# google/yggdrasil-decision-forests

Measured on NVIDIA H100. Metric: GBT boosting iters/sec, 10M rows x 200 num feats, higher is better.
Workload: dtype int64 fixed-point sums (q24 gradients), f64 split scores

## Files before the change

include/ygg_b200.h:

```cpp
#ifndef YGG_B200_H_
#define YGG_B200_H_

#include <stdint.h>

#ifdef __cplusplus
extern "C" {
#endif

#define YGG_ABI_VERSION 3

enum ygg_status {
  YGG_OK = 0,
  YGG_ERR_INVALID_ARGUMENT = 1,
  YGG_ERR_NO_DEVICE = 2,
  YGG_ERR_CUDA = 3,
  YGG_ERR_UNIMPLEMENTED = 4,
  YGG_ERR_CANCELLED = 5,
  YGG_ERR_IO = 6
};

enum ygg_loss {
  YGG_LOSS_BINOMIAL_LOG_LIKELIHOOD = 0,
  YGG_LOSS_SQUARED_ERROR = 1,
  YGG_LOSS_MULTINOMIAL_LOG_LIKELIHOOD = 2
// ... 40 lines not shown
  YGG_FEATURE_DISCRETIZED_NUMERICAL = 0,
  YGG_FEATURE_CATEGORICAL = 1,
  YGG_FEATURE_NUMERICAL = 2
};

typedef struct ygg_node {
  int32_t feature;
  int32_t threshold_bin;
  int32_t na_value;
  int32_t depth;
  int32_t neg_child;
  int32_t pos_child;
  float split_score;
  float leaf_value;
  int64_t num_examples;
  int64_t num_pos_examples;
  double stat[3];
  int32_t condition_type;
  float threshold_value;
  uint32_t cat_mask[8];
} ygg_node;

typedef struct ygg_dataset ygg_dataset;
typedef struct ygg_gbt ygg_gbt;

int ygg_abi_version(void);
const char* ygg_last_error(void);
int ygg_device_count(void);

int ygg_dataset_create(ygg_dataset** out, int64_t n_rows, int32_t n_features,
                       const uint8_t* bins, int64_t column_stride,
                       const int32_t* num_bins, const int32_t* na_bin, int32_t device);
int ygg_dataset_set_feature_types(ygg_dataset* ds, const int32_t* feature_types, int32_t n_features);
int ygg_dataset_set_bucket_values(ygg_dataset* ds, int32_t feature, const float* values, int32_t n, float na_replacement);
int ygg_dataset_set_wide_column(ygg_dataset* ds, int32_t feature, const uint16_t* codes, int64_t n, int32_t num_bins, int32_t na_bin,
                                const float* values, float na_replacement);
int ygg_dataset_set_wide_categorical_column(ygg_dataset* ds, int32_t feature, const uint16_t* codes, int64_t n, int32_t num_bins,
                                            int32_t na_bin);
int ygg_dataset_set_wide_discretized_column(ygg_dataset* ds, int32_t feature, const uint16_t* codes, int64_t n, int32_t num_bins,
                                            int32_t na_bin);
int ygg_dataset_get_wide_column(const ygg_dataset* ds, int32_t feature, uint16_t* codes, int32_t* num_bins, int32_t* na_bin);
int ygg_dataset_set_numerical_column(ygg_dataset* ds, int32_t feature, const float* values, int64_t n, float na_replacement);
int ygg_dataset_get_numerical_column(const ygg_dataset* ds, int32_t feature, float* values);
int ygg_dataset_destroy(ygg_dataset* ds);
int64_t ygg_dataset_num_rows(const ygg_dataset* ds);
int32_t ygg_dataset_num_features(const ygg_dataset* ds);

void ygg_gbt_config_init(ygg_gbt_config* cfg);
int ygg_gbt_create(ygg_gbt** out, ygg_dataset* ds, const ygg_gbt_config* cfg);
int ygg_gbt_destroy(ygg_gbt* h);

int ygg_gbt_set_labels_i32(ygg_gbt* h, const int32_t* labels, int64_t n);
int ygg_gbt_set_labels_f32(ygg_gbt* h, const float* labels, int64_t n);

int ygg_gbt_set_weights_f32(ygg_gbt* h, const float* weights, int64_t n);

int ygg_validation_split_mask(uint32_t random_seed, int64_t n_rows, float validation_ratio,
                              uint8_t* out_in_training );
int ygg_dataset_split_rows(const ygg_dataset* ds, const uint8_t* select, ygg_dataset** selected,
                           ygg_dataset** rest);
int ygg_gbt_set_validation_i32(ygg_gbt* h, const ygg_dataset* valid, const int32_t* labels, int64_t n);
int ygg_gbt_set_validation_f32(ygg_gbt* h, const ygg_dataset* valid, const float* labels, int64_t n);
int ygg_gbt_set_validation_weights_f32(ygg_gbt* h, const float* weights, int64_t n);
int ygg_gbt_validation_loss(ygg_gbt* h, int32_t iter, float* loss, float* secondary);
int32_t ygg_gbt_num_iterations(const ygg_gbt* h);
int ygg_gbt_final_validation(ygg_gbt* h, float* validation_loss, int32_t* early_stopping_triggered);

typedef int (*ygg_allgather_fn)(void* ctx, const void* send, void* recv, int64_t bytes,
                                void* stream);
int ygg_gbt_set_feature_shard(ygg_gbt* h, int32_t feature_begin, int32_t feature_end,
                              int32_t rank, int32_t world, ygg_allgather_fn exchange, void* ctx);

typedef int (*ygg_allreduce_fn)(void* ctx, void* buf, int64_t count, int32_t dtype, int32_t op, void* stream);
int ygg_gbt_set_row_shard(ygg_gbt* h, int32_t rank, int32_t world, int64_t n_rows_global,
                          float initial_prediction, ygg_allreduce_fn allreduce, void* ctx);

typedef int (*ygg_reducescatter_fn)(void* ctx, void* buf, int64_t count_per_rank, int32_t dtype, int32_t op,
                                    void* stream);
int ygg_gbt_set_row_shard_scatter(ygg_gbt* h, int32_t rank, int32_t world, int64_t n_rows_global,
                                  float initial_prediction, ygg_allreduce_fn allreduce,
                                  ygg_reducescatter_fn reducescatter, ygg_allgather_fn allgather, void* ctx);

int ygg_feature_shard(int32_t n_features, int32_t rank, int32_t world, int32_t* begin, int32_t* end);

typedef struct ygg_shard_best {
  float score;
  int32_t feature;
  int32_t threshold_bin;
  int32_t num_pos_examples;
  int32_t condition_type;
  int32_t na_value;
  uint32_t cat_mask[8];
} ygg_shard_best;
int ygg_merge_shard_best(const ygg_shard_best* records, int32_t world, int32_t nodes, ygg_shard_best* out);

int ygg_gbt_initial_prediction(ygg_gbt* h, float* out);

int ygg_gbt_train(ygg_gbt* h, int32_t num_iters, const volatile int32_t* stop_flag);
int ygg_gbt_step(ygg_gbt* h);
int ygg_gbt_sync(ygg_gbt* h);

int ygg_gbt_train_timed(ygg_gbt* h, int32_t num_iters, double* device_ms, int64_t* kernel_launches);

int32_t ygg_gbt_num_trees(const ygg_gbt* h);
int64_t ygg_gbt_best_split_window_bytes(const ygg_gbt* h);
int ygg_gbt_set_best_split_window(ygg_gbt* h, void* const* peer_windows, int32_t world);

int ygg_gbt_tie_stats(ygg_gbt* h, int64_t* renamed, int64_t* unresolved);
int ygg_gbt_set_tie_rng_position(ygg_gbt* h, uint64_t words);

int ygg_num_candidate_attributes(int32_t num_features, int32_t loss, int32_t num_candidate_attributes,
                                 float num_candidate_attributes_ratio, int32_t* k);
uint64_t ygg_candidate_key(uint32_t random_seed, int32_t tree, int32_t node, int32_t feature);
int ygg_gbt_set_candidate_sampling(ygg_gbt* h, int32_t num_candidate_attributes, float num_candidate_attributes_ratio);

int ygg_gbt_set_dart(ygg_gbt* h, float dropout_rate);
int ygg_gbt_get_dart_weights(ygg_gbt* h, float* out, int32_t capacity, int32_t* n);
int ygg_gbt_get_dart_dropped(ygg_gbt* h, int32_t iter, int32_t* out, int32_t capacity, int32_t* n);

int ygg_gbt_get_tree(ygg_gbt* h, int32_t iter, ygg_node* out, int32_t capacity, int32_t* n_nodes);
int ygg_gbt_get_category_set(ygg_gbt* h, int32_t iter, int32_t node, uint32_t* words, int32_t capacity, int32_t* n_words);
int ygg_gbt_train_loss(ygg_gbt* h, int32_t iter, float* loss, float* secondary);
int ygg_gbt_get_predictions(ygg_gbt* h, float* out, int64_t n);
int ygg_gbt_predict(ygg_gbt* h, const ygg_dataset* ds, float* out, int64_t n);

int ygg_gbt_set_predictions(ygg_gbt* h, const float* pred, int64_t n);

int ygg_tree_train_on_gradients(ygg_gbt* h, const float* gradients, const float* hessians,
                                ygg_node* out, int32_t capacity, int32_t* n_nodes);

enum ygg_hist_mode {
  YGG_HIST_ROOT_SUM = 0,
  YGG_HIST_PACKED = 1,
  YGG_HIST_SHARED = 2,
  YGG_HIST_HIST2 = 3,
  YGG_HIST_SEGMENTED = 4,
};
typedef struct ygg_hist_plan {
  int32_t mode;
  int32_t group;
  union {
    int32_t hist2_tiles;
    int32_t root_lanes;
  };
  int32_t chunk_blocks;
  int32_t slot_window;
  int32_t grid;
} ygg_hist_plan;
int ygg_debug_hist_plan(const ygg_gbt* h, int32_t level, ygg_hist_plan* out);
int ygg_debug_level_histogram(ygg_gbt* h, int32_t level, const ygg_hist_plan* plan, const float* gradients,
                              const float* second, const int32_t* slot_of_row, int32_t n_slots, uint64_t* out_sum,
                              uint32_t* out_cnt, uint64_t* out_second, float* out_scales);

int ygg_debug_wide_histogram(ygg_gbt* h, int32_t n_slots, uint64_t* out_sum, uint32_t* out_cnt, uint64_t* out_second);

int ygg_debug_capture_candidates(ygg_gbt* h, int32_t enabled);
typedef struct ygg_level_node {
  int32_t node;
  int32_t candidate;
  int32_t derived;
  int32_t reserved;
  int64_t num_examples;
} ygg_level_node;
typedef struct ygg_candidate {
  int32_t found;
  float score;
  int32_t threshold_bin;
  int32_t lo, hi;
  int32_t num_pos_examples;
  float threshold_value;
  uint32_t cat_mask[8];
} ygg_candidate;
int ygg_debug_level_candidates(ygg_gbt* h, int32_t level, int32_t capacity, ygg_level_node* nodes, ygg_candidate* cands,
                               uint32_t* sets, int32_t set_words, int32_t* n_nodes, float* scales);
int ygg_debug_level_tried(ygg_gbt* h, int32_t level, int32_t capacity, uint8_t* tried, int32_t* first_node, int32_t* n_nodes);

int ygg_partition_rows(ygg_dataset* ds, const uint32_t* rows_in, int64_t n, int32_t feature,
                       int32_t threshold_bin, uint32_t* rows_out, int64_t* n_pos);

int ygg_gbt_set_profiling(ygg_gbt* h, int32_t enabled);
int ygg_gbt_get_profile(ygg_gbt* h, const char* name, double* ms, int64_t* launches);

int ygg_gbt_save_ydf(ygg_gbt* h, const char* directory, const char* label_name,
                     const uint8_t* data_spec_pb, int64_t data_spec_len, int32_t label_col_idx,
                     const int32_t* feature_col_idx);

#ifdef __cplusplus
}
#endif
#endif
```

yggdrasil-decision-forests_b200/_capi.py:

```python
import ctypes as C
import os

import numpy as np

from . import _build

_LIB = None


class YggError(RuntimeError):
    def __init__(self, code, msg):
        super().__init__(f"[ygg status {code}] {msg}")
        self.code = code


class GbtConfig(C.Structure):
    _fields_ = [
        ("abi_version", C.c_int32), ("loss", C.c_int32), ("num_trees", C.c_int32),
        ("shrinkage", C.c_float), ("max_depth", C.c_int32), ("min_examples", C.c_int32),
        ("in_split_min_examples_check", C.c_int32), ("use_hessian_gain", C.c_int32),
        ("l1_regularization", C.c_float), ("l2_regularization", C.c_float),
        ("l2_regularization_categorical", C.c_float), ("clamp_leaf_logit", C.c_float),
        ("hessian_split_score_subtract_parent", C.c_int32), ("random_seed", C.c_uint32),
        ("subsample", C.c_float), ("validation_ratio", C.c_float),
        ("sibling_subtraction", C.c_int32), ("early_stopping", C.c_int32),
        ("early_stopping_num_trees_look_ahead", C.c_int32), ("early_stopping_initial_iteration", C.c_int32),
        ("num_classes", C.c_int32), ("candidate_shuffle", C.c_int32), ("rng_words_consumed", C.c_uint32),
        ("split_jobs_draw_seeds", C.c_int32), ("growing_strategy", C.c_int32), ("max_num_nodes", C.c_int32),
        ("goss_alpha", C.c_float), ("goss_beta", C.c_float),
    ]


NODE_DTYPE = np.dtype([
    ("feature", "<i4"), ("threshold_bin", "<i4"), ("na_value", "<i4"), ("depth", "<i4"),
    ("neg_child", "<i4"), ("pos_child", "<i4"), ("split_score", "<f4"), ("leaf_value", "<f4"),
    ("num_examples", "<i8"), ("num_pos_examples", "<i8"), ("stat", "<f8", (3,)),
    ("condition_type", "<i4"), ("threshold_value", "<f4"), ("cat_mask", "<u4", (8,)),
])
assert NODE_DTYPE.itemsize == 112

FEATURE_DISCRETIZED_NUMERICAL = 0
FEATURE_CATEGORICAL = 1
FEATURE_NUMERICAL = 2

LEVEL_NODE_DTYPE = np.dtype([("node", "<i4"), ("candidate", "<i4"), ("derived", "<i4"), ("reserved", "<i4"),
                             ("num_examples", "<i8")])
assert LEVEL_NODE_DTYPE.itemsize == 24
CANDIDATE_DTYPE = np.dtype([("found", "<i4"), ("score", "<f4"), ("threshold_bin", "<i4"), ("lo", "<i4"), ("hi", "<i4"),
                            ("num_pos_examples", "<i4"), ("threshold_value", "<f4"), ("cat_mask", "<u4", (8,))])
assert CANDIDATE_DTYPE.itemsize == 60

HIST_ROOT_SUM, HIST_PACKED, HIST_SHARED, HIST2, HIST_SEGMENTED = 0, 1, 2, 3, 4


class HistPlan(C.Structure):
    _fields_ = [("mode", C.c_int32), ("group", C.c_int32), ("hist2_tiles", C.c_int32), ("chunk_blocks", C.c_int32),
                ("slot_window", C.c_int32), ("grid", C.c_int32)]

    root_lanes = property(lambda self: self.hist2_tiles, lambda self, v: setattr(self, "hist2_tiles", v))

    def __repr__(self):
        return "HistPlan(%s)" % ", ".join("%s=%d" % (k, getattr(self, k)) for k, _ in self._fields_)

ALLGATHER_FN = C.CFUNCTYPE(C.c_int, C.c_void_p, C.c_void_p, C.c_void_p, C.c_int64, C.c_void_p)
ALLREDUCE_FN = C.CFUNCTYPE(C.c_int, C.c_void_p, C.c_void_p, C.c_int64, C.c_int32, C.c_int32, C.c_void_p)
REDUCESCATTER_FN = C.CFUNCTYPE(C.c_int, C.c_void_p, C.c_void_p, C.c_int64, C.c_int32, C.c_int32, C.c_void_p)

EXPORTS = [
    "ygg_abi_version", "ygg_last_error", "ygg_device_count", "ygg_dataset_create",
    "ygg_dataset_set_feature_types", "ygg_dataset_destroy", "ygg_dataset_num_rows", "ygg_dataset_num_features",
    "ygg_gbt_config_init", "ygg_gbt_create", "ygg_gbt_destroy", "ygg_gbt_set_labels_i32",
    "ygg_gbt_set_labels_f32", "ygg_gbt_set_weights_f32", "ygg_gbt_set_validation_weights_f32", "ygg_gbt_set_feature_shard", "ygg_gbt_set_row_shard", "ygg_gbt_set_row_shard_scatter", "ygg_feature_shard",
    "ygg_merge_shard_best", "ygg_gbt_initial_prediction",
    "ygg_gbt_train", "ygg_gbt_train_timed", "ygg_gbt_step", "ygg_gbt_sync", "ygg_gbt_num_trees", "ygg_gbt_get_tree",
    "ygg_gbt_train_loss", "ygg_gbt_get_predictions", "ygg_gbt_set_predictions", "ygg_gbt_predict",
    "ygg_tree_train_on_gradients", "ygg_debug_hist_plan", "ygg_debug_level_histogram", "ygg_partition_rows",
    "ygg_gbt_set_profiling", "ygg_gbt_get_profile", "ygg_gbt_save_ydf",
    "ygg_discretize_boundaries", "ygg_discretize_encode", "ygg_model_write_ydf",
    "ygg_validation_split_mask", "ygg_dataset_split_rows", "ygg_gbt_set_validation_i32",
    "ygg_gbt_set_validation_f32", "ygg_gbt_validation_loss", "ygg_gbt_num_iterations", "ygg_gbt_final_validation",
    "ygg_gen_discretized_boundaries", "ygg_dataset_builder_create", "ygg_dataset_builder_add_numerical",
    "ygg_dataset_builder_add_numerical_async", "ygg_dataset_builder_get_numerical",
    "ygg_dataset_builder_add_bins", "ygg_dataset_builder_finish", "ygg_dataset_builder_destroy",
    "ygg_dataset_get_bins", "ygg_dataset_set_bucket_values", "ygg_gbt_tie_stats", "ygg_gbt_set_tie_rng_position",
    "ygg_gbt_best_split_window_bytes", "ygg_gbt_set_best_split_window", "ygg_comm_window_create",
    "ygg_comm_unique_id", "ygg_comm_create", "ygg_comm_destroy", "ygg_comm_allreduce", "ygg_comm_allgather", "ygg_comm_reducescatter",
    "ygg_dataset_set_wide_column", "ygg_dataset_get_wide_column", "ygg_debug_wide_histogram",
    "ygg_dataset_set_wide_categorical_column", "ygg_gbt_get_category_set",
    "ygg_dataset_set_numerical_column", "ygg_dataset_get_numerical_column",
    "ygg_debug_capture_candidates", "ygg_debug_level_candidates",
    "ygg_num_candidate_attributes", "ygg_candidate_key", "ygg_gbt_set_candidate_sampling", "ygg_debug_level_tried",
    "ygg_gbt_set_dart", "ygg_gbt_get_dart_weights", "ygg_gbt_get_dart_dropped",
    "ygg_dataset_set_wide_discretized_column", "ygg_dataset_builder_add_numerical16_async", "ygg_discretize_boundaries16",
]


def lib():
    global _LIB
    if _LIB is None:
        path = _build.build()
        L = C.CDLL(path)
        L.ygg_last_error.restype = C.c_char_p
        L.ygg_dataset_num_rows.restype = C.c_int64
        L.ygg_gbt_config_init.restype = None
        L.ygg_candidate_key.restype = C.c_uint64
        L.ygg_candidate_key.argtypes = [C.c_uint32, C.c_int32, C.c_int32, C.c_int32]
        for name in EXPORTS:
            getattr(L, name)
        _LIB = L
    return _LIB


def check(status):
    if status != 0:
        raise YggError(status, lib().ygg_last_error().decode("utf-8", "replace"))


def ptr(a, t):
    return a.ctypes.data_as(C.POINTER(t)) if a is not None else None


def num_candidate_attributes(num_features, loss, num_candidate_attributes=-1, ratio=None):
    k = C.c_int32()
    check(lib().ygg_num_candidate_attributes(C.c_int32(int(num_features)), C.c_int32(int(loss)),
                                             C.c_int32(int(num_candidate_attributes)),
                                             C.c_float(-1.0 if ratio is None else float(ratio)), C.byref(k)))
    return k.value


def candidate_key(seed, tree, node, feature):
    return int(lib().ygg_candidate_key(int(seed) & 0xFFFFFFFF, int(tree), int(node), int(feature)))


def default_config(**kw):
    cfg = GbtConfig()
    lib().ygg_gbt_config_init(C.byref(cfg))
    for k, v in kw.items():
        if not hasattr(cfg, k):
            raise AttributeError(k)
        setattr(cfg, k, v)
    return cfg


class Dataset:

    def __init__(self, bins, num_bins, na_bin, device=0, feature_types=None):
        b = np.asarray(bins)
        if not (b.dtype == np.uint8 and b.ndim == 2 and b.strides[1] == 1 and b.strides[0] >= b.shape[1]):
            b = np.ascontiguousarray(bins, dtype=np.uint8)
        assert b.ndim == 2, "bins must be [n_features, n_rows] (column-major storage)"
        self.n_features, self.n_rows = b.shape
        self.num_bins = np.ascontiguousarray(num_bins, dtype=np.int32)
        self.na_bin = np.ascontiguousarray(na_bin, dtype=np.int32)
        assert len(self.num_bins) == self.n_features and len(self.na_bin) == self.n_features
        self.handle = C.c_void_p()
        self.h2d_bytes = self.n_features * self.n_rows
        col_stride = b.strides[0] if self.n_features > 1 else max(int(b.strides[0]), self.n_rows)
        check(lib().ygg_dataset_create(C.byref(self.handle), C.c_int64(self.n_rows),
                                       C.c_int32(self.n_features), C.cast(b.ctypes.data, C.POINTER(C.c_uint8)),
                                       C.c_int64(col_stride), ptr(self.num_bins, C.c_int32),
                                       ptr(self.na_bin, C.c_int32), C.c_int32(device)))
        self.feature_types = np.zeros(self.n_features, np.int32)
        if feature_types is not None:
            self.set_feature_types(feature_types)

    def set_bucket_values(self, feature, values, na_replacement):
        v = np.ascontiguousarray(values, dtype=np.float32)
        check(lib().ygg_dataset_set_bucket_values(self.handle, C.c_int32(int(feature)), ptr(v, C.c_float), C.c_int32(len(v)),
                                                  C.c_float(float(np.float32(na_replacement)))))

    def set_wide_column(self, feature, codes, num_bins, na_bin, values, na_replacement):
        c = np.ascontiguousarray(codes, dtype=np.uint16)
        v = np.ascontiguousarray(values, dtype=np.float32)
        if len(v) != int(num_bins):
            raise ValueError(f"{len(v)} bucket values for {num_bins} buckets")
        check(lib().ygg_dataset_set_wide_column(self.handle, C.c_int32(int(feature)), ptr(c, C.c_uint16), C.c_int64(len(c)),
                                                C.c_int32(int(num_bins)), C.c_int32(int(na_bin)), ptr(v, C.c_float),
                                                C.c_float(float(np.float32(na_replacement)))))
        self.num_bins = self.num_bins.copy()
        self.na_bin = self.na_bin.copy()
        self.num_bins[feature], self.na_bin[feature] = 1, 0
        self.wide = dict(getattr(self, "wide", {}))
        self.wide[int(feature)] = (int(num_bins), int(na_bin))

    def set_wide_categorical_column(self, feature, codes, num_bins, na_bin):
        c = np.ascontiguousarray(codes, dtype=np.uint16)
        check(lib().ygg_dataset_set_wide_categorical_column(self.handle, C.c_int32(int(feature)), ptr(c, C.c_uint16),
                                                            C.c_int64(len(c)), C.c_int32(int(num_bins)), C.c_int32(int(na_bin))))
        self.num_bins = self.num_bins.copy()
        self.na_bin = self.na_bin.copy()
        self.num_bins[feature], self.na_bin[feature] = 1, 0
        self.wide = dict(getattr(self, "wide", {}))
        self.wide[int(feature)] = (int(num_bins), int(na_bin))

    def set_wide_discretized_column(self, feature, codes, num_bins, na_bin):
        c = np.ascontiguousarray(codes, dtype=np.uint16)
        check(lib().ygg_dataset_set_wide_discretized_column(self.handle, C.c_int32(int(feature)), ptr(c, C.c_uint16),
                                                            C.c_int64(len(c)), C.c_int32(int(num_bins)), C.c_int32(int(na_bin))))
        self.num_bins = self.num_bins.copy()
        self.na_bin = self.na_bin.copy()
        self.num_bins[feature], self.na_bin[feature] = 1, 0
        self.wide = dict(getattr(self, "wide", {}))
        self.wide[int(feature)] = (int(num_bins), int(na_bin))

    def get_wide_column(self, feature):
        out = np.empty(self.n_rows, np.uint16)
        nb, na = C.c_int32(), C.c_int32()
        check(lib().ygg_dataset_get_wide_column(self.handle, C.c_int32(int(feature)), ptr(out, C.c_uint16), C.byref(nb), C.byref(na)))
        return out, nb.value, na.value

    def set_numerical_column(self, feature, values, na_replacement):
        v = np.ascontiguousarray(values, dtype=np.float32)
        check(lib().ygg_dataset_set_numerical_column(self.handle, C.c_int32(int(feature)), ptr(v, C.c_float), C.c_int64(len(v)),
                                                     C.c_float(float(np.float32(na_replacement)))))
        self.num_bins = self.num_bins.copy()
        self.na_bin = self.na_bin.copy()
        self.num_bins[feature], self.na_bin[feature] = 1, 0
        self.feature_types = self.feature_types.copy()
        self.feature_types[feature] = FEATURE_NUMERICAL

    def get_numerical_column(self, feature):
        out = np.empty(self.n_rows, np.float32)
        check(lib().ygg_dataset_get_numerical_column(self.handle, C.c_int32(int(feature)), ptr(out, C.c_float)))
        return out

    def set_feature_types(self, feature_types):
        ft = np.ascontiguousarray(feature_types, dtype=np.int32)
        check(lib().ygg_dataset_set_feature_types(self.handle, ptr(ft, C.c_int32), C.c_int32(len(ft))))
        self.feature_types = ft

    def close(self):
        if self.handle:
            lib().ygg_dataset_destroy(self.handle)
            self.handle = C.c_void_p()

    def split_rows(self, select):
        m = np.ascontiguousarray(select, dtype=np.uint8)
        assert m.shape == (self.n_rows,)
        a, b = C.c_void_p(), C.c_void_p()
        check(lib().ygg_dataset_split_rows(self.handle, ptr(m, C.c_uint8), C.byref(a), C.byref(b)))
        out = []
        for hnd, n in ((a, int(m.astype(bool).sum())), (b, int(len(m) - m.astype(bool).sum()))):
            d = Dataset.__new__(Dataset)
            d.handle, d.n_features, d.n_rows = hnd, self.n_features, n
            d.num_bins, d.na_bin, d.feature_types, d.h2d_bytes = self.num_bins, self.na_bin, self.feature_types, 0
            d.wide = dict(getattr(self, "wide", {}))
# ... 278 lines not shown
                        return int(fn(*a) or 0)
                    except Exception:
                        import traceback
                        traceback.print_exc()
                        return 1
                return _cb
            self._cbs = (ALLREDUCE_FN(wrap(allreduce, 5)), REDUCESCATTER_FN(wrap(reducescatter, 5)),
                         ALLGATHER_FN(wrap(allgather, 4)))
            fns, ctx = self._cbs, None
        check(lib().ygg_gbt_set_row_shard_scatter(self.handle, C.c_int32(rank), C.c_int32(world),
                                                  C.c_int64(n_rows_global), C.c_float(initial_prediction),
                                                  fns[0], fns[1], fns[2], ctx))

    def set_row_shard(self, rank, world, n_rows_global, initial_prediction, allreduce=None):
        if isinstance(allreduce, Comm):
            self._comm = allreduce
            fn = C.cast(lib().ygg_comm_allreduce, ALLREDUCE_FN)
            check(lib().ygg_gbt_set_row_shard(self.handle, C.c_int32(rank), C.c_int32(world),
                                              C.c_int64(n_rows_global), C.c_float(initial_prediction), fn,
                                              allreduce.handle))
            return
        if allreduce is not None:
            def _cb(ctx, buf, count, dtype, op, stream):
                try:
                    return int(allreduce(buf, count, dtype, op, stream) or 0)
                except Exception:
                    import traceback
                    traceback.print_exc()
                    return 1
            self._cb = ALLREDUCE_FN(_cb)
            fn = self._cb
        else:
            fn = C.cast(None, ALLREDUCE_FN)
        check(lib().ygg_gbt_set_row_shard(self.handle, C.c_int32(rank), C.c_int32(world),
                                          C.c_int64(n_rows_global), C.c_float(initial_prediction), fn, None))

    def initial_prediction(self):
        v = C.c_float()
        check(lib().ygg_gbt_initial_prediction(self.handle, C.byref(v)))
        return v.value

    def train(self, num_iters, stop_flag=None):
        check(lib().ygg_gbt_train(self.handle, C.c_int32(num_iters), stop_flag))

    def train_timed(self, num_iters):
        ms, n = C.c_double(), C.c_int64()
        check(lib().ygg_gbt_train_timed(self.handle, C.c_int32(num_iters), C.byref(ms), C.byref(n)))
        return ms.value, n.value

    def step(self):
        check(lib().ygg_gbt_step(self.handle))

    def sync(self):
        check(lib().ygg_gbt_sync(self.handle))

    def num_trees(self):
        return int(lib().ygg_gbt_num_trees(self.handle))

    def use_peer_windows(self, comm):
        L = lib()
        L.ygg_gbt_best_split_window_bytes.restype = C.c_int64
        nbytes = int(L.ygg_gbt_best_split_window_bytes(self.handle))
        peers = (C.c_void_p * comm.world)()
        check(L.ygg_comm_window_create(comm.handle, C.c_int64(nbytes), peers))
        check(L.ygg_gbt_set_best_split_window(self.handle, peers, C.c_int32(comm.world)))

    def set_tie_rng_position(self, words):
        check(lib().ygg_gbt_set_tie_rng_position(self.handle, C.c_uint64(int(words))))

    def tie_stats(self):
        a, b = C.c_int64(), C.c_int64()
        check(lib().ygg_gbt_tie_stats(self.handle, C.byref(a), C.byref(b)))
        return a.value, b.value

    def get_tree(self, it):
        cap = (1 << (self.cfg.max_depth + (1 if self.cfg.growing_strategy == 1 else 0)))
        out = np.zeros(cap, dtype=NODE_DTYPE)
        n = C.c_int32()
        check(lib().ygg_gbt_get_tree(self.handle, C.c_int32(it), out.ctypes.data_as(C.c_void_p),
                                     C.c_int32(cap), C.byref(n)))
        return out[:n.value].copy()

    def get_category_sets(self, it, tree=None):
        wide = getattr(self.dataset, "wide", {})
        if not wide:
            return {}
        t = self.get_tree(it) if tree is None else tree
        out = {}
        for i in np.flatnonzero((t["condition_type"] == FEATURE_CATEGORICAL) & (t["feature"] >= 0)):
            f = int(t["feature"][i])
            if f not in wide:
                continue
            words = np.zeros((wide[f][0] + 31) // 32, np.uint32)
            n = C.c_int32()
            check(lib().ygg_gbt_get_category_set(self.handle, C.c_int32(it), C.c_int32(int(i)), ptr(words, C.c_uint32),
                                                 C.c_int32(len(words)), C.byref(n)))
            out[int(i)] = words
        return out

    def train_loss(self, it):
        a, b = C.c_float(), C.c_float()
        check(lib().ygg_gbt_train_loss(self.handle, C.c_int32(it), C.byref(a), C.byref(b)))
        return a.value, b.value

    def get_predictions(self):
        k = self.cfg.num_classes if self.cfg.loss == 2 else 1
        out = np.empty(self.dataset.n_rows * k, dtype=np.float32)
        check(lib().ygg_gbt_get_predictions(self.handle, ptr(out, C.c_float), C.c_int64(len(out))))
        return out if k == 1 else np.ascontiguousarray(out.reshape(k, self.dataset.n_rows).T)

    def predict(self, dataset):
        n = int(lib().ygg_dataset_num_rows(dataset.handle))
        K = int(self.cfg.num_classes) if self.cfg.loss == 2 else 1
        out = np.empty(n * K, dtype=np.float32)
        check(lib().ygg_gbt_predict(self.handle, dataset.handle, ptr(out, C.c_float), C.c_int64(n * K)))
        return out if K == 1 else np.ascontiguousarray(out.reshape(K, n).T)

    def set_predictions(self, pred):
        p = np.ascontiguousarray(pred, dtype=np.float32)
        check(lib().ygg_gbt_set_predictions(self.handle, ptr(p, C.c_float), C.c_int64(len(p))))

    def train_tree_on_gradients(self, g, h=None):
        g = np.ascontiguousarray(g, dtype=np.float32)
        h = None if h is None else np.ascontiguousarray(h, dtype=np.float32)
        cap = (1 << (self.cfg.max_depth + (1 if self.cfg.growing_strategy == 1 else 0)))
        out = np.zeros(cap, dtype=NODE_DTYPE)
        n = C.c_int32()
        check(lib().ygg_tree_train_on_gradients(self.handle, ptr(g, C.c_float), ptr(h, C.c_float),
                                                out.ctypes.data_as(C.c_void_p), C.c_int32(cap),
                                                C.byref(n)))
        return out[:n.value].copy()

    def hist_plan(self, level):
        p = HistPlan()
        check(lib().ygg_debug_hist_plan(self.handle, C.c_int32(level), C.byref(p)))
        return p

    def level_histogram(self, level, g, slot_of_row, n_slots, second=None, plan=None):
        g = np.ascontiguousarray(g, dtype=np.float32)
        slots = np.ascontiguousarray(slot_of_row, dtype=np.int32)
        v = None if second is None else np.ascontiguousarray(second, dtype=np.float32)
        lo, hi = self.hist_features()
        shape = (int(n_slots), hi - lo, 256)
        s = np.zeros(shape, np.uint64)
        c = np.zeros(shape, np.uint32)
        s2 = None if v is None else np.zeros(shape, np.uint64)
        scales = np.zeros(2, np.float32)
        check(lib().ygg_debug_level_histogram(self.handle, C.c_int32(level), None if plan is None else C.byref(plan),
                                              ptr(g, C.c_float), ptr(v, C.c_float), ptr(slots, C.c_int32),
                                              C.c_int32(n_slots), ptr(s, C.c_uint64), ptr(c, C.c_uint32),
                                              ptr(s2, C.c_uint64), ptr(scales, C.c_float)))
        return s, c, s2, (float(scales[0]), float(scales[1]))

    def wide_histogram(self, n_slots):
        total = sum(nb for nb, _ in getattr(self.dataset, "wide", {}).values())
        s = np.zeros((int(n_slots), total), np.uint64)
        c = np.zeros((int(n_slots), total), np.uint32)
        s2 = np.zeros((int(n_slots), total), np.uint64) if self.has_second_plane() else None
        check(lib().ygg_debug_wide_histogram(self.handle, C.c_int32(int(n_slots)), ptr(s, C.c_uint64), ptr(c, C.c_uint32),
                                             ptr(s2, C.c_uint64)))
        return s, c, s2

    def has_second_plane(self):
        weighted = getattr(self, "_weighted", False) or self.cfg.goss_alpha > 0 or self.cfg.goss_beta > 0
        logit = self.cfg.loss in (0, 2)
        return bool((self.cfg.use_hessian_gain and (logit or weighted)) or weighted)

    def debug_histogram(self, g, node_of_row, node, feature):
        lo, hi = self.hist_features()
        if not lo <= feature < hi:
            raise ValueError(f"feature {feature} outside the histogrammed features [{lo}, {hi})")
        slots = np.where(np.asarray(node_of_row) == node, 0, -1).astype(np.int32)
        root = self.hist_plan(0)
        p = HistPlan(HIST_SHARED, 1, 0, root.chunk_blocks, 0, root.grid)
        second = np.zeros(len(slots), np.float32) if self.has_second_plane() else None
        s, c, _, (P, _) = self.level_histogram(0, g, slots, 1, second=second, plan=p)
        nb = int(self.dataset.num_bins[feature])
        cnt = c[0, feature - lo, :nb].astype(np.int64)
        raw = s[0, feature - lo, :nb].astype(np.int64) - cnt * 2 ** 23
        return raw.astype(np.float64) * (P / 2.0 ** 23), cnt

    def set_candidate_sampling(self, num_candidate_attributes=-1, ratio=None):
        check(lib().ygg_gbt_set_candidate_sampling(self.handle, C.c_int32(int(num_candidate_attributes)),
                                                   C.c_float(-1.0 if ratio is None else float(ratio))))

    def set_dart(self, dropout_rate):
        check(lib().ygg_gbt_set_dart(self.handle, C.c_float(float(dropout_rate))))

    def dart_weights(self):
        n = C.c_int32()
        cap = int(self.cfg.num_trees)
        out = np.zeros(max(cap, 1), np.float32)
        check(lib().ygg_gbt_get_dart_weights(self.handle, ptr(out, C.c_float), C.c_int32(cap), C.byref(n)))
        return out[:n.value].copy()

    def dart_dropped(self, it):
        n = C.c_int32()
        out = np.zeros(max(int(it), 1), np.int32)
        check(lib().ygg_gbt_get_dart_dropped(self.handle, C.c_int32(int(it)), ptr(out, C.c_int32), C.c_int32(len(out)),
                                             C.byref(n)))
        return out[:n.value].copy()

    def level_tried(self, level):
        cap = 1 << max(0, self.cfg.max_depth - 1)
        lo, hi = self.hist_features()
        out = np.zeros((cap, hi - lo), np.uint8)
        first, n = C.c_int32(), C.c_int32()
        check(lib().ygg_debug_level_tried(self.handle, C.c_int32(int(level)), C.c_int32(cap), ptr(out, C.c_uint8),
                                          C.byref(first), C.byref(n)))
        return out[:n.value].copy(), first.value

    def capture_candidates(self, on=True):
        check(lib().ygg_debug_capture_candidates(self.handle, C.c_int32(int(bool(on)))))

    def level_candidates(self, level):
        cap = 1 << max(0, self.cfg.max_depth - 1)
        lo, hi = self.hist_features()
        nodes = np.zeros(cap, LEVEL_NODE_DTYPE)
        cands = np.zeros((cap, hi - lo), CANDIDATE_DTYPE)
        wide = getattr(self.dataset, "wide", {})
        words = max([(nb + 31) // 32 for f, (nb, _) in wide.items()
                     if self.dataset.feature_types[f] == FEATURE_CATEGORICAL] or [0])
        sets = np.zeros((cap, len(wide), words), np.uint32) if words else None
        n, scales = C.c_int32(), np.zeros(3, np.float32)
        check(lib().ygg_debug_level_candidates(self.handle, C.c_int32(int(level)), C.c_int32(cap),
                                               nodes.ctypes.data_as(C.c_void_p), cands.ctypes.data_as(C.c_void_p),
                                               ptr(sets, C.c_uint32), C.c_int32(words), C.byref(n), ptr(scales, C.c_float)))
        k = n.value
        out = {name: nodes[name][:k].copy() for name in ("node", "candidate", "derived", "num_examples")}
        out.update({name: cands[name][:k].copy() for name in CANDIDATE_DTYPE.names})
        if sets is not None:
            out["sets"] = sets[:k].copy()
        out["P"], out["h_pow2"], out["w_pow2"] = (float(x) for x in scales)
        return out

    def hist_features(self):
        return getattr(self, "_hist_features", (0, self.dataset.n_features))

    def set_profiling(self, enabled=True):
        check(lib().ygg_gbt_set_profiling(self.handle, C.c_int32(int(enabled))))

    def get_profile(self, name):
        ms, n = C.c_double(), C.c_int64()
        check(lib().ygg_gbt_get_profile(self.handle, name.encode(), C.byref(ms), C.byref(n)))
        return ms.value, n.value


SHARD_BEST_DTYPE = np.dtype([("score", "<f4"), ("feature", "<i4"), ("threshold_bin", "<i4"),
                             ("num_pos_examples", "<i4"), ("condition_type", "<i4"), ("na_value", "<i4"),
                             ("cat_mask", "<u4", (8,))])
assert SHARD_BEST_DTYPE.itemsize == 56


def feature_shard(n_features, rank, world):
    b, e = C.c_int32(), C.c_int32()
    check(lib().ygg_feature_shard(C.c_int32(n_features), C.c_int32(rank), C.c_int32(world),
                                  C.byref(b), C.byref(e)))
    return b.value, e.value


def merge_shard_best(records):
    r = np.ascontiguousarray(records, dtype=SHARD_BEST_DTYPE)
    world, nodes = r.shape
    out = np.zeros(nodes, dtype=SHARD_BEST_DTYPE)
    check(lib().ygg_merge_shard_best(r.ctypes.data_as(C.c_void_p), C.c_int32(world), C.c_int32(nodes),
                                     out.ctypes.data_as(C.c_void_p)))
    return out


def device_count():
    return int(lib().ygg_device_count())


def discretize_boundaries(values, maximum_num_bins=255, min_obs_in_bins=3):
    v = np.ascontiguousarray(values, dtype=np.float32)
    out = np.zeros(max(2, maximum_num_bins + 4), dtype=np.float32)
    n = C.c_int32()
    mean = C.c_double()
    check(lib().ygg_discretize_boundaries(ptr(v, C.c_float), C.c_int64(len(v)),
                                          C.c_int32(maximum_num_bins), C.c_int32(min_obs_in_bins),
                                          ptr(out, C.c_float), C.c_int32(len(out)), C.byref(n),
                                          C.byref(mean)))
    return out[:n.value].copy(), mean.value


def discretize_boundaries16(values, maximum_num_bins, min_obs_in_bins=3):
    v = np.ascontiguousarray(values, dtype=np.float32)
    out = np.zeros(maximum_num_bins + 4, dtype=np.float32)
    n = C.c_int32()
    mean = C.c_double()
    check(lib().ygg_discretize_boundaries16(ptr(v, C.c_float), C.c_int64(len(v)),
                                            C.c_int32(maximum_num_bins), C.c_int32(min_obs_in_bins),
                                            ptr(out, C.c_float), C.c_int32(len(out)), C.byref(n),
                                            C.byref(mean)))
    return out[:n.value].copy(), mean.value


def discretize_encode(values, boundaries, na_bin):
    v = np.ascontiguousarray(values, dtype=np.float32)
    b = np.ascontiguousarray(boundaries, dtype=np.float32)
    out = np.empty(len(v), dtype=np.uint8)
    check(lib().ygg_discretize_encode(ptr(v, C.c_float), C.c_int64(len(v)), ptr(b, C.c_float),
                                      C.c_int32(len(b)), C.c_int32(na_bin), ptr(out, C.c_uint8)))
    return out
```

yggdrasil-decision-forests_b200/csrc/ygg_engine.cu:

```cuda
#include <algorithm>
#include <mutex>
#include <random>
#include <cmath>
#include <cstdarg>
#include <cstdio>
#include <cstdlib>
#include <cstring>
#include <limits>
#include <map>
#include <queue>
#include <string>
#include <thread>
#include <vector>

#include <cuda_runtime.h>
#include <cub/device/device_radix_sort.cuh>
#include <cub/device/device_scan.cuh>
#include <nvtx3/nvToolsExt.h>

#include "../../include/ygg_b200.h"
#include "ygg_internal.h"
#include "../../include/ygg_b200_model.h"
#include "ygg_kernels.cuh"
#include "ygg_wide.cuh"
// ... 108 lines not shown
  float* d_pred = nullptr;
  float* d_g = nullptr;
  float* d_h = nullptr;
  uint32_t* d_q24 = nullptr;
  uint32_t* d_hq24 = nullptr;
  uint2* d_act = nullptr;
  uint32_t* d_act_h = nullptr;
  int32_t* d_act_count = nullptr;
  int32_t* d_act_sub = nullptr;
  uint32_t* d_root_cnt = nullptr;
  bool root_cnt_valid = false;
  int n_blocks = 0;
  uint16_t* d_node_of_row = nullptr;
  DeviceState* d_st = nullptr;
  LevelDesc* d_levels = nullptr;
  Family* d_fam[2] = {nullptr, nullptr};
  int32_t* d_slot_node[2] = {nullptr, nullptr};
  NodeRec* d_nodes_all = nullptr;
  NodeRec* d_nodes_scratch = nullptr;
  int tree_capacity = 0;
  unsigned long long* d_hist_sum[2] = {nullptr, nullptr};
  uint32_t* d_hist_cnt[2] = {nullptr, nullptr};
  unsigned long long* d_hist_hsum[2] = {nullptr, nullptr};
  Candidate* d_cand = nullptr;
  uint32_t* d_cand_mask = nullptr;
  int64_t wide_total = 0;
  int wide_slots = 0;
  bool counted = false;
  unsigned long long* d_wsum = nullptr;
  uint32_t* d_wcnt = nullptr;
  unsigned long long* d_whsum = nullptr;
  unsigned long long* d_wnode_sum[2] = {nullptr, nullptr};
  uint32_t* d_wnode_cnt[2] = {nullptr, nullptr};
  unsigned long long* d_wnode_hsum[2] = {nullptr, nullptr};
  float* d_wide_thr = nullptr;
  int32_t* d_wide_feature = nullptr;
  int32_t* d_wide_bins = nullptr;
  int32_t* d_wide_disc = nullptr;
  int set_words = 0;
  int64_t sort_total = 0;
  int64_t* d_sort_off = nullptr;
  int32_t* d_wide_cat = nullptr;
  int32_t* d_wide_na_bin = nullptr;
  uint32_t* d_wide_set = nullptr;
  double* d_sort_key = nullptr;
  int32_t* d_sort_idx = nullptr;
  uint32_t* d_sets = nullptr;
  float* d_master_val = nullptr;
  uint32_t* d_master_row = nullptr;
  float* d_list_val[2] = {nullptr, nullptr};
  uint32_t* d_list_row[2] = {nullptr, nullptr};
  unsigned long long* d_ps = nullptr;
  unsigned long long* d_ph = nullptr;
  int64_t* d_seg_off = nullptr;
  int64_t* d_seg_total = nullptr;
  unsigned long long* d_sbest = nullptr;
  unsigned long long* d_sbest_idx = nullptr;
  int32_t* d_num_feature = nullptr;
  void* d_presort_temp = nullptr;
  size_t presort_temp_bytes = 0;
  bool scratch_tree = false;
  ShardBest* d_shard_best = nullptr;
  TieRec* d_ties = nullptr;
  int sample_k_valid = 0;
  uint8_t* d_tried = nullptr;
  bool dart = false;
  float dart_rate = 0.f;
  uint16_t* d_dart_hist = nullptr;
  uint16_t* d_dart_vhist = nullptr;
  float* d_dart_leaf = nullptr;
  DartDrop* d_dart_list[2] = {nullptr, nullptr};
  std::vector<std::vector<int32_t>> dart_dropped;
  std::vector<float> dart_w_new, dart_sf_m1, dart_w;
  std::vector<DartDrop> dart_host_list;
  struct Capture {
    bool on = false;
    int levels = 0;
    const NodeRec* tree = nullptr;
    int f_scan = 0;
    size_t nodes = 0, set_elems = 0;
    Candidate* cand = nullptr;
    uint32_t* mask = nullptr;
    float* thr = nullptr;
    uint32_t* set = nullptr;
    uint8_t* tried = nullptr;
    NodeRec* node_tab = nullptr;
    Family* fam = nullptr;
    LevelDesc* lv = nullptr;
    DeviceState* st = nullptr;
  } cap;
  uint8_t* d_selected = nullptr;
  std::vector<uint8_t> host_selected;
  int64_t n_selected = 0;
  std::mt19937 tie_rng;
  bool tie_rng_ready = false;
  int ties_resolved_upto = 0;
  int64_t ties_renamed = 0, ties_unresolved = 0;
  LossRec* d_loss = nullptr;
  LossPartials* d_loss_partials = nullptr;
  unsigned long long* d_level_buf = nullptr;
  size_t level_buf_bytes = 0;
  size_t slot_elems_cap = 0;
  int stats_cap = 0;
  int shard_mode = kShardNone;
  int hist_f_begin = 0, hist_f_end = 0;
  int64_t n_global = 0;
  ygg_allreduce_fn allreduce = nullptr;
  ygg_reducescatter_fn reducescatter = nullptr;
  bool scatter = false;
  int loss_reduced_upto = 0;
  int max_nodes = 0, max_level_nodes = 0, num_levels = 0;
  int trees_done = 0;
  bool pending = false;
  int K = 1;
  int iters_done = 0;
  bool pending_loss = false;
  float* cur_g = nullptr;
  float* cur_h = nullptr;
  float* cur_g2w = nullptr;
  const ygg_dataset* vds = nullptr;
  float* d_vpred = nullptr;
  uint8_t* d_vlabel_u8 = nullptr;
  float* d_vlabel_f32 = nullptr;
  LossRec* d_vloss = nullptr;
  float* d_weight = nullptr;
  float* d_g2w = nullptr;
  unsigned long long* d_wsums = nullptr;
  std::vector<float> host_weights;
  double sum_weights = 0;
  float w_pow2 = 1.f;
  float* d_goss_keys[2] = {nullptr, nullptr};
  uint32_t* d_goss_rows[2] = {nullptr, nullptr};
  float* d_goss_u = nullptr;
  void* d_goss_temp = nullptr;
  size_t goss_temp_bytes = 0;
  std::vector<float> host_goss_u;
  int64_t goss_cutoff = 0;
  float* d_vweight = nullptr;
  double v_sum_weights = 0;
  float v_correct_scale = 0.f;
  bool finalized = false;
  int final_trees = -1;
  int log_entries = -1;
  float final_validation_loss = 0.f;
  bool early_stopping_triggered = false;
  int f_begin = 0, f_end = 0, rank = 0, world = 1;
  ygg_allgather_fn exchange = nullptr;
  void* exchange_ctx = nullptr;
  void** d_peer_windows = nullptr;
  uint32_t exchange_epoch = 0;
  HistLaunch hist_plan[32]{};
  int part_smem_children = 0;
  uint2* d_hseg = nullptr;
  long long* d_hseg_blk = nullptr;
  long long* d_hseg_off = nullptr;
  int32_t* d_hseg_piece = nullptr;
  int32_t* d_hseg_meta = nullptr;
  void* d_hseg_temp = nullptr;
  size_t hseg_temp_bytes = 0;
  bool profiling = false;
  std::map<std::string, ProfileSlot> profile;
  std::vector<std::pair<std::string, std::pair<cudaEvent_t, cudaEvent_t>>> pending_events;
  int64_t launches_total = 0;
};

namespace {

bool use_hess(const ygg_gbt* h) { return h->cfg.use_hessian_gain != 0; }
bool is_logit(const ygg_gbt* h) {
  return h->cfg.loss == YGG_LOSS_BINOMIAL_LOG_LIKELIHOOD || h->cfg.loss == YGG_LOSS_MULTINOMIAL_LOG_LIKELIHOOD;
}
bool is_multinomial(const ygg_gbt* h) { return h->cfg.loss == YGG_LOSS_MULTINOMIAL_LOG_LIKELIHOOD; }
bool weighted(const ygg_gbt* h) { return h->d_weight != nullptr; }
bool has_h(const ygg_gbt* h) { return is_logit(h) || weighted(h); }
float h_pow2_of(const ygg_gbt* h) { return (is_logit(h) ? 0.25f : 1.f) * (weighted(h) ? h->w_pow2 : 1.f); }
float correct_scale_of(float w_pow2) { return static_cast<float>(1u << kSBits) / w_pow2; }
bool hist_hess(const ygg_gbt* h) { return (use_hess(h) && has_h(h)) || weighted(h); }
bool goss(const ygg_gbt* h) { return h->cfg.goss_alpha > 0.f || h->cfg.goss_beta > 0.f; }
bool sampling(const ygg_gbt* h) { return h->cfg.subsample < 1.f - std::numeric_limits<float>::epsilon() || goss(h); }
bool user_weighted(const ygg_gbt* h) { return h->d_weight != nullptr && !goss(h); }

inline bool nvtx_enabled() {
  static const bool on = [] { const char* v = std::getenv("YGG_NVTX"); return v != nullptr && std::atoi(v) != 0; }();
  return on;
}
struct ProfScope {
  ygg_gbt* h;
  const char* name;
  cudaEvent_t a = nullptr, b = nullptr;
  ProfScope(ygg_gbt* h_, const char* n) : h(h_), name(n) {
    if (nvtx_enabled()) nvtxRangePushA(n);
    if (h->profiling) {
      cudaEventCreate(&a);
      cudaEventCreate(&b);
      cudaEventRecord(a, h->stream);
    }
  }
  ~ProfScope() {
    if (h->profiling) {
      cudaEventRecord(b, h->stream);
      h->pending_events.push_back({name, {a, b}});
    }
    if (nvtx_enabled()) nvtxRangePop();
  }
};

void collect_profile(ygg_gbt* h) {
  for (auto& e : h->pending_events) {
    float ms = 0;
    cudaEventSynchronize(e.second.second);
    cudaEventElapsedTime(&ms, e.second.first, e.second.second);
    auto& s = h->profile[e.first];
    s.ms += ms;
    s.launches++;
    cudaEventDestroy(e.second.first);
    cudaEventDestroy(e.second.second);
  }
  h->pending_events.clear();
}

int check_launch(const char* what) {
  cudaError_t e = cudaGetLastError();
  if (e != cudaSuccess) return set_error(YGG_ERR_CUDA, "launch of %s failed: %s", what, cudaGetErrorString(e));
  return YGG_OK;
}

int level_slot_bound(const ygg_gbt* h, int level) {
  if (level == 0) return 1;
  return h->cfg.sibling_subtraction ? (1 << (level - 1)) : (1 << level);
}

struct LevelBuf {
  unsigned long long* sum;
  unsigned long long* hsum;
  uint32_t* cnt;
  unsigned long long* stats;
  int W;
  int f_chunk;
  size_t chunk_u64;
  size_t planes_u64;
  size_t total_u64;
};
LevelBuf level_buf(const ygg_gbt* h, int slots, int n_stats_nodes, unsigned long long* base = nullptr) {
  LevelBuf lb;
  const int f_hist = h->hist_f_end - h->hist_f_begin;
  lb.W = h->scatter ? h->world : 1;
  lb.f_chunk = (f_hist + lb.W - 1) / lb.W;
  const size_t B = static_cast<size_t>(slots) * lb.f_chunk * kMaxBins;
  if (base == nullptr) base = h->d_level_buf;
  lb.sum = base;
  unsigned long long* p = lb.sum + B;
  lb.hsum = nullptr;
  if (hist_hess(h)) { lb.hsum = p; p += B; }
  lb.cnt = reinterpret_cast<uint32_t*>(p);
  p += (B + 1) / 2;
  lb.stats = p;
  lb.planes_u64 = static_cast<size_t>(p - base);
  p += static_cast<size_t>(n_stats_nodes) * 3;
  lb.chunk_u64 = static_cast<size_t>(p - base);
  lb.total_u64 = lb.chunk_u64 * lb.W;
  return lb;
}

__global__ void k_zero_planes(unsigned long long* base, size_t chunk_u64, size_t planes_u64) {
  unsigned long long* c = base + static_cast<size_t>(blockIdx.y) * chunk_u64;
  for (size_t i = static_cast<size_t>(blockIdx.x) * blockDim.x + threadIdx.x; i < planes_u64;
       i += static_cast<size_t>(gridDim.x) * blockDim.x)
    c[i] = 0ull;
}
__global__ void k_replicate_stats(unsigned long long* stats0, size_t chunk_u64, int n_words, int W) {
  const int i = blockIdx.x * blockDim.x + threadIdx.x;
  if (i >= n_words) return;
  const unsigned long long v = stats0[i];
  for (int c = 1; c < W; c++) stats0[static_cast<size_t>(c) * chunk_u64 + i] = v;
}

int zero_planes(ygg_gbt* h, const LevelBuf& lb) {
  if (lb.W == 1) {
    YGG_CUDA(cudaMemsetAsync(lb.sum, 0, lb.planes_u64 * sizeof(unsigned long long), h->stream));
    return YGG_OK;
  }
  dim3 grid(static_cast<unsigned>(std::min<size_t>((lb.planes_u64 + 255) / 256, 1024)), static_cast<unsigned>(lb.W));
  k_zero_planes<<<grid, 256, 0, h->stream>>>(lb.sum, lb.chunk_u64, lb.planes_u64);
  h->launches_total++;
  return check_launch("k_zero_planes");
}
int replicate_stats(ygg_gbt* h, const LevelBuf& lb, int n_nodes) {
  if (lb.W == 1) return YGG_OK;
  k_replicate_stats<<<(3 * n_nodes + 127) / 128, 128, 0, h->stream>>>(lb.stats, lb.chunk_u64, 3 * n_nodes, lb.W);
  h->launches_total++;
  return check_launch("k_replicate_stats");
}

template <typename F>
int for_hist_kernel(bool hess, int mode, F f, bool multi = false) {
  if (multi) {
    if (hess) return f(k_hist<true, kHistShared, true>);
    if (mode == kHistPacked) return f(k_hist<false, kHistPacked, true>);
    return f(k_hist<false, kHistShared, true>);
  }
  if (hess) return f(k_hist<true, kHistShared>);
  if (mode == kHistRootSum) return f(k_hist<false, kHistRootSum>);
  if (mode == kHistPacked) return f(k_hist<false, kHistPacked>);
  return f(k_hist<false, kHistShared>);
}

int hist_smem_budget(int device, size_t* budget) {
  int optin = 0;
  YGG_CUDA(cudaDeviceGetAttribute(&optin, cudaDevAttrMaxSharedMemoryPerBlockOptin, device));
  cudaFuncAttributes fa{};
  YGG_CUDA(cudaFuncGetAttributes(&fa, k_hist<false, kHistPacked>));
  *budget = static_cast<size_t>(optin) - fa.sharedSizeBytes;
  return YGG_OK;
}
constexpr size_t kHist2SmemBudget = 216 * 1024;

int sub_blocks_of(const ygg_gbt* h) { return h->ds->n_pad / kBlockRows >= 512 ? 8 : 1; }
int chunk_max_count(ygg_gbt* h, int chunk_blocks, uint32_t** d_sub, uint32_t* out_max) {
  const int kSubBlocks = sub_blocks_of(h);
  const ygg_dataset* ds = h->ds;
  const int f_count = h->hist_f_end - h->hist_f_begin;
  const int n_blocks = static_cast<int>(ds->n_pad / kBlockRows);
  const int n_subs = (n_blocks + kSubBlocks - 1) / kSubBlocks;
  if (*d_sub == nullptr) {
    YGG_RETURN_IF_ERROR(dev_alloc(d_sub, static_cast<size_t>(n_subs) * f_count * kMaxBins + 1));
    k_sub_counts<<<dim3(n_subs, f_count), 256>>>(ds->d_bins, ds->n, ds->n_pad, h->hist_f_begin, kSubBlocks, *d_sub);
    YGG_RETURN_IF_ERROR(check_launch("k_sub_counts"));
  }
  uint32_t* d_max = *d_sub + static_cast<size_t>(n_subs) * f_count * kMaxBins;
  YGG_CUDA(cudaMemset(d_max, 0, sizeof(uint32_t)));
  const int subs_per_chunk = chunk_blocks / kSubBlocks;
  const int n_chunks = (n_subs + subs_per_chunk - 1) / subs_per_chunk;
  k_chunk_max<<<dim3(n_chunks, f_count), 256>>>(*d_sub, n_subs, subs_per_chunk, d_max);
  YGG_CUDA(cudaMemcpy(out_max, d_max, sizeof(uint32_t), cudaMemcpyDeviceToHost));
  return YGG_OK;
}

int raise_hist_smem_caps_once(int device) {
  static std::mutex mu;
  static std::vector<char> done;
  std::lock_guard<std::mutex> lock(mu);
  if (static_cast<int>(done.size()) <= device) done.resize(device + 1, 0);
  if (done[device]) return YGG_OK;
  size_t budget = 0;
  YGG_RETURN_IF_ERROR(hist_smem_budget(device, &budget));
  auto set_cap = [](size_t bytes) {
    return [bytes](auto kern) -> int {
      YGG_CUDA(cudaFuncSetAttribute(kern, cudaFuncAttributeMaxDynamicSharedMemorySize, static_cast<int>(bytes)));
      return YGG_OK;
    };
  };
  for (const bool hess : {false, true})
    for (const int mode : {kHistRootSum, kHistPacked, kHistShared})
      for (const bool multi : {false, true}) YGG_RETURN_IF_ERROR(for_hist_kernel(hess, mode, set_cap(budget), multi));
  const auto cap2 = set_cap(kHist2SmemBudget);
  YGG_RETURN_IF_ERROR(cap2(k_hist2<32, true>)); YGG_RETURN_IF_ERROR(cap2(k_hist2<32, false>));
  YGG_RETURN_IF_ERROR(cap2(k_hist2<16, true>)); YGG_RETURN_IF_ERROR(cap2(k_hist2<16, false>));
  YGG_RETURN_IF_ERROR(cap2(k_hist2<8, true>)); YGG_RETURN_IF_ERROR(cap2(k_hist2<8, false>));
  YGG_RETURN_IF_ERROR(set_cap(seg_smem_bytes(64))(k_hist_seg<32, 2>));
  YGG_RETURN_IF_ERROR(set_cap(seg_smem_bytes(32))(k_hist_seg<32, 1>));
  YGG_RETURN_IF_ERROR(set_cap(seg_smem_bytes(16))(k_hist_seg<16, 1>));
  YGG_RETURN_IF_ERROR(set_cap(seg_smem_bytes(8))(k_hist_seg<8, 1>));
  YGG_CUDA(cudaFuncSetAttribute(k_hist_seg<32, 2>, cudaFuncAttributePreferredSharedMemoryCarveout, cudaSharedmemCarveoutMaxShared));
  YGG_CUDA(cudaFuncSetAttribute(k_hist_seg<32, 1>, cudaFuncAttributePreferredSharedMemoryCarveout, cudaSharedmemCarveoutMaxShared));
  YGG_CUDA(cudaFuncSetAttribute(k_hist_seg<16, 1>, cudaFuncAttributePreferredSharedMemoryCarveout, cudaSharedmemCarveoutMaxShared));
  YGG_CUDA(cudaFuncSetAttribute(k_hist_seg<8, 1>, cudaFuncAttributePreferredSharedMemoryCarveout, cudaSharedmemCarveoutMaxShared));
  YGG_RETURN_IF_ERROR(set_cap(kRootSmemBytes)(k_hist_root_rows));
  done[device] = 1;
  return YGG_OK;
}

int configure_launches(ygg_gbt* h) {
  (void)cudaGetLastError();
  const bool hh = hist_hess(h);
  size_t budget = 0;
// ... 267 lines not shown
                                             h->d_master_row + static_cast<int64_t>(p) * n, static_cast<int>(n), 0, 32, h->stream));
  YGG_CUDA(cudaStreamSynchronize(h->stream));
  return YGG_OK;
}

PresortParams presort_params(ygg_gbt* h, NodeRec* nodes, int l, const ScanParams& sc) {
  const ygg_dataset* ds = h->ds;
  PresortParams p{};
  p.s = sc; p.level = l; p.P = ds->n_num(); p.n = ds->n; p.num_feature = h->d_num_feature;
  const bool master = l == 0 && !sampling(h);
  p.val = master ? h->d_master_val : h->d_list_val[l & 1];
  p.row = master ? h->d_master_row : h->d_list_row[l & 1];
  p.s.nodes = nodes; p.s.levels = h->d_levels;
  p.node_of_row = h->d_node_of_row; p.seg_off = h->d_seg_off; p.seg_total = h->d_seg_total;
  p.q24 = h->d_q24; p.hq24 = hist_hess(h) ? h->d_hq24 : nullptr; p.ps = h->d_ps; p.ph = h->d_ph;
  p.best = h->d_sbest; p.best_idx = h->d_sbest_idx; p.thr_value = h->d_wide_thr;
  return p;
}

int presort_scan(ygg_gbt* h, const PresortParams& p) {
  const int64_t total = static_cast<int64_t>(p.P) * p.n;
  const int grid = elementwise_grid(h);
  if (p.level == 0) {
    k_presort_segments<<<1, 1024, 0, h->stream>>>(h->d_levels, p.s.nodes, 0, h->d_seg_off, h->d_seg_total);
    h->launches_total++;
    YGG_RETURN_IF_ERROR(check_launch("k_presort_segments"));
    if (sampling(h)) {
      uint32_t* flags = reinterpret_cast<uint32_t*>(h->d_ps);
      k_presort_sample_flags<<<grid, 256, 0, h->stream>>>(h->d_master_row, total, h->d_selected, flags);
      YGG_CUDA(cub::DeviceScan::ExclusiveSum(h->d_presort_temp, h->presort_temp_bytes, flags, flags, total, h->stream));
      k_presort_sample_scatter<<<grid, 256, 0, h->stream>>>(h->d_master_val, h->d_master_row, p.n, total, h->d_selected, flags,
                                                            h->d_list_val[0], h->d_list_row[0]);
      h->launches_total += 3;
      YGG_RETURN_IF_ERROR(check_launch("k_presort_sample_scatter"));
    }
  }
  k_presort_gather<<<grid, 256, 0, h->stream>>>(p);
  YGG_CUDA(cub::DeviceScan::InclusiveSum(h->d_presort_temp, h->presort_temp_bytes, h->d_ps, h->d_ps, total, h->stream));
  if (p.hq24 != nullptr)
    YGG_CUDA(cub::DeviceScan::InclusiveSum(h->d_presort_temp, h->presort_temp_bytes, h->d_ph, h->d_ph, total, h->stream));
  const size_t slots = (static_cast<size_t>(1) << p.level) * p.P;
  YGG_CUDA(cudaMemsetAsync(h->d_sbest, 0, slots * sizeof(unsigned long long), h->stream));
  YGG_CUDA(cudaMemsetAsync(h->d_sbest_idx, 0xFF, slots * sizeof(unsigned long long), h->stream));
  if (hist_hess(h) || use_hess(h)) {
    k_presort_scan<true, true><<<grid, 256, 0, h->stream>>>(p);
    k_presort_scan<true, false><<<grid, 256, 0, h->stream>>>(p);
  } else {
    k_presort_scan<false, true><<<grid, 256, 0, h->stream>>>(p);
    k_presort_scan<false, false><<<grid, 256, 0, h->stream>>>(p);
  }
  k_presort_candidates<<<static_cast<unsigned>((slots + 255) / 256), 256, 0, h->stream>>>(p);
  h->launches_total += 5 + (p.hq24 != nullptr ? 1 : 0);
  return check_launch("k_presort_candidates");
}

int presort_partition(ygg_gbt* h, NodeRec* nodes, int l) {
  ScanParams sc{};
  PresortParams p = presort_params(h, nodes, l, sc);
  const int64_t total = static_cast<int64_t>(p.P) * p.n;
  const int grid = elementwise_grid(h);
  k_presort_segments<<<1, 1024, 0, h->stream>>>(h->d_levels, nodes, l + 1, h->d_seg_off, h->d_seg_total);
  uint32_t* flags = reinterpret_cast<uint32_t*>(h->d_ps);
  k_presort_flags<<<grid, 256, 0, h->stream>>>(p, flags);
  YGG_CUDA(cub::DeviceScan::ExclusiveSum(h->d_presort_temp, h->presort_temp_bytes, flags, flags, total, h->stream));
  k_presort_scatter<<<grid, 256, 0, h->stream>>>(p, flags, h->d_list_val[(l + 1) & 1], h->d_list_row[(l + 1) & 1]);
  h->launches_total += 4;
  return check_launch("k_presort_scatter");
}

int allocate_level_buffers(ygg_gbt* h) {
  const int f_scan = h->f_end - h->f_begin;
  const int f_hist = h->hist_f_end - h->hist_f_begin;
  for (int i = 0; i < 2; i++) {
    dev_free(h->d_hist_sum[i]); dev_free(h->d_hist_cnt[i]); dev_free(h->d_hist_hsum[i]);
    h->d_hist_sum[i] = nullptr; h->d_hist_cnt[i] = nullptr; h->d_hist_hsum[i] = nullptr;
  }
  dev_free(h->d_cand); h->d_cand = nullptr;
  dev_free(h->d_cand_mask); h->d_cand_mask = nullptr;
  cudaFree(h->d_level_buf); h->d_level_buf = nullptr;
  const size_t split_level_nodes = static_cast<size_t>(1) << std::max(0, h->num_levels - 1);
  const size_t node_elems = split_level_nodes * f_scan * kMaxBins;
  for (int i = 0; i < 2; i++) {
    YGG_RETURN_IF_ERROR(dev_alloc(&h->d_hist_sum[i], node_elems));
    YGG_RETURN_IF_ERROR(dev_alloc(&h->d_hist_cnt[i], node_elems));
    if (hist_hess(h)) YGG_RETURN_IF_ERROR(dev_alloc(&h->d_hist_hsum[i], node_elems));
  }
  YGG_RETURN_IF_ERROR(dev_alloc(&h->d_cand, split_level_nodes * f_scan));
  YGG_RETURN_IF_ERROR(dev_alloc(&h->d_cand_mask, split_level_nodes * f_scan * 8));
  if (h->d_shard_best == nullptr)
    YGG_RETURN_IF_ERROR(dev_alloc_plain(&h->d_shard_best, static_cast<size_t>(std::max(1, h->world)) * h->max_level_nodes));
  size_t max_u64 = 16;
  for (int l = 0; l <= h->num_levels; l++) {
    const int slots = l < h->num_levels ? level_slot_bound(h, l) : 0;
    const int stats_nodes = l == 0 ? 1 : (2 << (l - 1));
    max_u64 = std::max(max_u64, level_buf(h, slots, stats_nodes).total_u64);
  }
  (void)f_hist;
  h->level_buf_bytes = max_u64 * sizeof(unsigned long long);
  YGG_RETURN_IF_ERROR(dev_alloc_plain(&h->d_level_buf, max_u64));
  return allocate_wide_buffers(h);
}

int launch_hist(ygg_gbt* h, const HistParams& hp, int mode, int grid, size_t smem, bool multi = false) {
  return for_hist_kernel(hist_hess(h), mode, [&](auto kern) -> int {
    kern<<<grid, kHistThreads, smem, h->stream>>>(hp);
    h->launches_total++;
    return check_launch("k_hist");
  }, multi);
}

int ensure_bins4(ygg_dataset* ds) {
  if (ds->d_bins4 != nullptr) return YGG_OK;
  const int groups = (ds->F + 3) / 4;
  YGG_RETURN_IF_ERROR(dev_alloc(&ds->d_bins4, static_cast<size_t>(groups) * ds->n_pad));
  dim3 grid(static_cast<unsigned>(std::min<int64_t>((ds->n_pad / 4 + 255) / 256, 4096)), static_cast<unsigned>(groups));
  k_interleave4<<<grid, 256>>>(ds->d_bins, ds->n_pad, ds->F, ds->d_bins4);
  YGG_RETURN_IF_ERROR(check_launch("k_interleave4"));
  YGG_CUDA(cudaDeviceSynchronize());
  return YGG_OK;
}

int launch_hist2(ygg_gbt* h, const Hist2Params& hp, int FL, bool root, int grid) {
  const size_t smem = hist2_smem_bytes(FL, hp.S, hp.T, root);
  auto go = [&](auto kern) -> int {
    kern<<<grid, kHist2Threads, smem, h->stream>>>(hp);
    h->launches_total++;
    return check_launch("k_hist2");
  };
  if (FL == 32) return root ? go(k_hist2<32, true>) : go(k_hist2<32, false>);
  if (FL == 16) return root ? go(k_hist2<16, true>) : go(k_hist2<16, false>);
  return root ? go(k_hist2<8, true>) : go(k_hist2<8, false>);
}

int ensure_bins_rows(ygg_dataset* ds) {
  static std::mutex mu;
  std::lock_guard<std::mutex> lock(mu);
  if (ds->d_bins_rows != nullptr) return YGG_OK;
  const int row_bytes = seg_row_bytes(ds->F);
  uint8_t* rows = nullptr;
  YGG_RETURN_IF_ERROR(dev_alloc(&rows, static_cast<size_t>(row_bytes) * ds->n_pad));
  dim3 grid(static_cast<unsigned>((ds->n_pad + 255) / 256), static_cast<unsigned>(row_bytes / 32));
  k_bins_to_rows<<<grid, 256>>>(ds->d_bins, ds->n_pad, ds->F, row_bytes, rows);
  int st = check_launch("k_bins_to_rows");
  if (st == YGG_OK && cudaDeviceSynchronize() != cudaSuccess) st = set_error(YGG_ERR_CUDA, "k_bins_to_rows failed");
  if (st != YGG_OK) {
    dev_free(rows);
    return st;
  }
  ds->d_bins_rows = rows;
  return YGG_OK;
}

void free_seg_buffers(ygg_gbt* h) {
  dev_free(h->d_hseg); dev_free(h->d_hseg_blk); dev_free(h->d_hseg_off); dev_free(h->d_hseg_piece); dev_free(h->d_hseg_meta);
  dev_free(h->d_hseg_temp);
  h->d_hseg = nullptr; h->d_hseg_blk = nullptr; h->d_hseg_off = nullptr; h->d_hseg_piece = nullptr; h->d_hseg_meta = nullptr;
  h->d_hseg_temp = nullptr;
  h->hseg_temp_bytes = 0;
}
int ensure_seg_buffers(ygg_gbt* h) {
  if (h->d_hseg_temp != nullptr) return YGG_OK;
  const size_t ranges = static_cast<size_t>(kSegMaxSlots) * h->n_blocks;
  auto alloc_all = [&]() -> int {
    YGG_RETURN_IF_ERROR(dev_alloc(&h->d_hseg, static_cast<size_t>(h->ds->n_pad)));
    YGG_RETURN_IF_ERROR(dev_alloc(&h->d_hseg_blk, ranges));
    YGG_RETURN_IF_ERROR(dev_alloc(&h->d_hseg_off, ranges + 1));
    YGG_RETURN_IF_ERROR(dev_alloc(&h->d_hseg_piece, ranges + 1));
    YGG_RETURN_IF_ERROR(dev_alloc(&h->d_hseg_meta, 4));
    size_t temp_bytes = 0;
    YGG_CUDA(cub::DeviceScan::InclusiveSum(nullptr, temp_bytes, h->d_hseg_blk, h->d_hseg_blk, static_cast<int>(ranges)));
    char* temp = nullptr;
    YGG_RETURN_IF_ERROR(dev_alloc(&temp, temp_bytes));
    h->hseg_temp_bytes = temp_bytes;
    h->d_hseg_temp = temp;
    return YGG_OK;
  };
  const int st = alloc_all();
  if (st != YGG_OK) free_seg_buffers(h);
  return st;
}

int launch_hist_seg(ygg_gbt* h, int l, const LevelBuf& lb, const LevelDesc* levels, const HistLaunch& pl) {
  ygg_dataset* ds = h->ds;
  YGG_RETURN_IF_ERROR(ensure_bins_rows(ds));
  YGG_RETURN_IF_ERROR(ensure_seg_buffers(h));
  const int f_count = h->hist_f_end - h->hist_f_begin;
  const int n_chunks = (h->n_blocks + pl.chunk - 1) / pl.chunk;
  const int fpl = seg_lane_features(pl.SL, f_count);
  const int n_fg = seg_feature_groups(pl.SL, fpl, h->hist_f_begin, f_count);
  const int target_pieces = std::max(1, (kSegItemsPerCta * pl.grid + n_fg - 1) / n_fg);
  k_seg_count<<<std::min(h->n_blocks, ds->num_sms * 8), 256, 0, h->stream>>>(h->d_act, h->d_act_count, h->n_blocks, pl.S,
                                                                               levels, l, h->d_hseg_blk);
  YGG_RETURN_IF_ERROR(check_launch("k_seg_count"));
  YGG_CUDA(cub::DeviceScan::InclusiveSum(h->d_hseg_temp, h->hseg_temp_bytes, h->d_hseg_blk, h->d_hseg_blk, pl.S * h->n_blocks,
                                         h->stream));
  k_seg_ranges<<<1, kSegScanThreads, 0, h->stream>>>(h->d_hseg_blk, pl.S, h->n_blocks, pl.chunk, n_chunks, target_pieces,
                                                     h->d_hseg_off, h->d_hseg_piece, h->d_hseg_meta);
  YGG_RETURN_IF_ERROR(check_launch("k_seg_ranges"));
  k_seg_scatter<<<std::min(h->n_blocks, ds->num_sms * 8), 256, 0, h->stream>>>(h->d_act, h->d_act_count, h->n_blocks, pl.S, levels, l,
                                                               h->d_hseg_blk, h->d_hseg);
  YGG_RETURN_IF_ERROR(check_launch("k_seg_scatter"));
  SegParams sp{};
  sp.rows = ds->d_bins_rows; sp.row_bytes = static_cast<uint32_t>(seg_row_bytes(ds->F));
  sp.seg = h->d_hseg; sp.seg_off = h->d_hseg_off; sp.piece_start = h->d_hseg_piece; sp.meta = h->d_hseg_meta;
  sp.n_ranges = pl.S * n_chunks; sp.n_chunks = n_chunks;
  sp.f_begin = h->hist_f_begin; sp.f_count = f_count;
  sp.hist_sum = lb.sum; sp.hist_cnt = lb.cnt;
  sp.f_chunk = lb.f_chunk; sp.chunk_stride = static_cast<long long>(lb.chunk_u64);
  const size_t smem = seg_smem_bytes(pl.SL * fpl);
  if (fpl == 2) k_hist_seg<32, 2><<<pl.grid, kSegThreads, smem, h->stream>>>(sp);
  else if (pl.SL == 32) k_hist_seg<32, 1><<<pl.grid, kSegThreads, smem, h->stream>>>(sp);
  else if (pl.SL == 16) k_hist_seg<16, 1><<<pl.grid, kSegThreads, smem, h->stream>>>(sp);
  else k_hist_seg<8, 1><<<pl.grid, kSegThreads, smem, h->stream>>>(sp);
  h->launches_total += 5;
  return check_launch("k_hist_seg");
}

int launch_hist_root_rows(ygg_gbt* h, const LevelBuf& lb, const HistLaunch& pl) {
  ygg_dataset* ds = h->ds;
  YGG_RETURN_IF_ERROR(ensure_bins_rows(ds));
  RootRowsParams rp{};
  rp.rows = ds->d_bins_rows; rp.row_bytes = static_cast<uint32_t>(seg_row_bytes(ds->F));
  rp.q24 = h->d_q24; rp.act_count = h->d_act_count; rp.n_blocks = h->n_blocks; rp.chunk_blocks = pl.chunk;
  rp.f_begin = h->hist_f_begin; rp.f_count = h->hist_f_end - h->hist_f_begin;
  rp.hist_sum = lb.sum; rp.f_chunk = lb.f_chunk; rp.chunk_stride = static_cast<long long>(lb.chunk_u64);
  k_hist_root_rows<<<pl.grid, kRootThreads, kRootSmemBytes, h->stream>>>(rp);
  h->launches_total++;
  return check_launch("k_hist_root_rows");
}

int ensure_root_counts(ygg_gbt* h) {
  if (h->root_cnt_valid) return YGG_OK;
  const int f_count = h->hist_f_end - h->hist_f_begin;
  if (h->d_root_cnt) dev_free(h->d_root_cnt);
  h->d_root_cnt = nullptr;
  const LevelBuf lb = level_buf(h, 1, 1);
  const size_t padded = static_cast<size_t>(lb.W) * lb.f_chunk * kMaxBins;
  YGG_RETURN_IF_ERROR(dev_alloc(&h->d_root_cnt, padded));
  YGG_CUDA(cudaMemsetAsync(h->d_root_cnt, 0, padded * sizeof(uint32_t), h->stream));
  dim3 grid(std::max(1, h->ds->num_sms * 8 / std::max(1, f_count)), f_count);
  k_root_counts<<<grid, 256, 0, h->stream>>>(h->ds->d_bins, h->ds->n, h->ds->n_pad, f_count, h->hist_f_begin, h->d_root_cnt);
  h->launches_total++;
  YGG_RETURN_IF_ERROR(check_launch("k_root_counts"));
  h->root_cnt_valid = true;
  return YGG_OK;
}

int accumulate_level(ygg_gbt* h, int l, const LevelBuf& lb, const LevelDesc* levels, const HistLaunch& pl) {
  const ygg_dataset* ds = h->ds;
  const int hist_f_count = h->hist_f_end - h->hist_f_begin;
  YGG_RETURN_IF_ERROR(zero_planes(h, lb));
  if (pl.mode == kHistRootSum) {
    const size_t row = static_cast<size_t>(lb.f_chunk) * kMaxBins * sizeof(uint32_t);
    YGG_CUDA(cudaMemcpy2DAsync(lb.cnt, lb.chunk_u64 * sizeof(unsigned long long), h->d_root_cnt, row, row, lb.W,
                               cudaMemcpyDeviceToDevice, h->stream));
  }
  if (pl.SL > 0) return launch_hist_seg(h, l, lb, levels, pl);
  if (pl.RL > 0) return launch_hist_root_rows(h, lb, pl);
  if (pl.FL > 0) {
    YGG_RETURN_IF_ERROR(ensure_bins4(h->ds));
    Hist2Params hp{};
    hp.bins4 = ds->d_bins4; hp.n_pad = ds->n_pad; hp.n = ds->n; hp.q24 = h->d_q24; hp.act = h->d_act;
    hp.act_count = h->d_act_count; hp.act_sub = h->d_act_sub; hp.n_blocks = h->n_blocks;
    hp.f_begin = h->hist_f_begin; hp.f_count = hist_f_count;
    hp.g_begin = h->hist_f_begin / 4; hp.n_groups = (h->hist_f_end + 3) / 4 - hp.g_begin;
    hp.S = pl.S; hp.T = pl.T; hp.chunk_blocks = pl.chunk;
    hp.level = l; hp.levels = levels;
    hp.hist_sum = lb.sum; hp.hist_cnt = lb.cnt;
    hp.f_chunk = lb.f_chunk; hp.chunk_stride = static_cast<long long>(lb.chunk_u64);
    return launch_hist2(h, hp, pl.FL, l == 0, pl.grid);
  }
  HistParams hp{};
  hp.bins = ds->d_bins; hp.n_pad = ds->n_pad; hp.act = h->d_act; hp.act_h = h->d_act_h; hp.q24 = h->d_q24;
  hp.act_count = h->d_act_count; hp.n_blocks = h->n_blocks;
  hp.f_begin = h->hist_f_begin; hp.f_count = hist_f_count; hp.G = pl.G; hp.S = pl.S;
  hp.chunk_blocks = pl.chunk;
  hp.level = l; hp.levels = levels;
  hp.hist_sum = lb.sum; hp.hist_cnt = lb.cnt; hp.hist_hsum = lb.hsum;
  hp.f_chunk = lb.f_chunk; hp.chunk_stride = static_cast<long long>(lb.chunk_u64);
  const size_t smem = hist_smem_bytes(pl.G, pl.S, hist_hess(h), pl.mode);
  if (pl.window > 0) {
    for (int pass = 0; pass < pl.passes; pass++) {
      hp.level = l | ((pass * pl.window) << 8) | (pl.window << 20);
      YGG_RETURN_IF_ERROR(launch_hist(h, hp, pl.mode, pl.grid, smem, true));
    }
    return YGG_OK;
  }
  return launch_hist(h, hp, pl.mode, pl.grid, smem);
}

int do_allreduce(ygg_gbt* h, void* buf, int64_t count, int dtype, int op) {
  if (h->allreduce == nullptr) return set_error(YGG_ERR_INVALID_ARGUMENT, "row sharding without an all-reduce function");
  const int rc = h->allreduce(h->exchange_ctx, buf, count, dtype, op, h->stream);
  if (rc != 0) return set_error(YGG_ERR_CUDA, "all-reduce failed with code %d", rc);
  return YGG_OK;
}

int launch_weight_sums(ygg_gbt* h, NodeRec* nodes) {
  ProfScope ps(h, "select");
  WeightSumParams wp{};
  wp.n = h->ds->n; wp.node_of_row = h->d_node_of_row; wp.selected = sampling(h) ? h->d_selected : nullptr;
  wp.weight = h->d_weight; wp.g2w = h->cur_g2w != nullptr ? h->cur_g2w : h->d_g2w; wp.st = h->d_st; wp.w_pow2 = h->w_pow2; wp.nodes = nodes;
  wp.sums = h->d_wsums; wp.levels = h->d_levels; wp.num_levels = h->num_levels + 1;
  wp.smem_nodes = h->max_nodes <= 2048 ? h->max_nodes : 0;
  YGG_CUDA(cudaMemsetAsync(h->d_wsums, 0, static_cast<size_t>(h->max_nodes) * 2 * sizeof(unsigned long long), h->stream));
  const size_t smem = static_cast<size_t>(wp.smem_nodes) * 2 * sizeof(unsigned long long);
  k_weight_sums_rows<<<h->ds->num_sms * 4, 256, smem, h->stream>>>(wp);
  if (h->shard_mode == kShardRows)
    YGG_RETURN_IF_ERROR(do_allreduce(h, h->d_wsums, static_cast<int64_t>(h->max_nodes) * 2, 1, 0));
  k_weight_sums_finish<<<1, 1024, 0, h->stream>>>(wp);
  h->launches_total += 2;
  return check_launch("k_weight_sums");
}

void free_capture(ygg_gbt* h) {
  dev_free(h->cap.cand); dev_free(h->cap.mask); dev_free(h->cap.thr); dev_free(h->cap.set); dev_free(h->cap.tried);
  dev_free(h->cap.node_tab); dev_free(h->cap.fam); dev_free(h->cap.lv); dev_free(h->cap.st);
  h->cap = ygg_gbt::Capture{};
}

int capture_level(ygg_gbt* h, int l, const NodeRec* nodes, int par) {
  ygg_gbt::Capture& c = h->cap;
  if (c.f_scan != h->f_end - h->f_begin)
    return set_error(YGG_ERR_INVALID_ARGUMENT, "the feature shard changed after ygg_debug_capture_candidates");
  const size_t per = c.nodes * c.f_scan;
  auto copy = [&](void* dst, const void* src, size_t bytes) {
    return cudaMemcpyAsync(dst, src, bytes, cudaMemcpyDeviceToDevice, h->stream);
  };
  YGG_CUDA(copy(c.cand + l * per, h->d_cand, per * sizeof(Candidate)));
  YGG_CUDA(copy(c.mask + l * per * 8, h->d_cand_mask, per * 8 * sizeof(uint32_t)));
  if (c.thr != nullptr) YGG_CUDA(copy(c.thr + l * per, h->d_wide_thr, per * sizeof(float)));
  if (c.set != nullptr) YGG_CUDA(copy(c.set + l * c.set_elems, h->d_wide_set, c.set_elems * sizeof(uint32_t)));
  if (c.tried != nullptr) YGG_CUDA(copy(c.tried + l * per, h->d_tried, per));
  YGG_CUDA(copy(c.node_tab + static_cast<size_t>(l) * h->max_nodes, nodes, h->max_nodes * sizeof(NodeRec)));
  YGG_CUDA(copy(c.fam + static_cast<size_t>(l) * h->max_level_nodes, h->d_fam[par], h->max_level_nodes * sizeof(Family)));
  YGG_CUDA(copy(c.lv + l, h->d_levels + l, sizeof(LevelDesc)));
  YGG_CUDA(copy(c.st, h->d_st, sizeof(DeviceState)));
  c.tree = nodes;
  c.levels = l + 1;
  return YGG_OK;
}

int grow_tree(ygg_gbt* h, NodeRec* nodes) {
  const ygg_dataset* ds = h->ds;
  const int f_count = h->f_end - h->f_begin;
  const int hist_f_count = h->hist_f_end - h->hist_f_begin;
  const bool rows_sharded = h->shard_mode == kShardRows;
  const int64_t n_job = sampling(h) ? h->n_selected : (rows_sharded ? h->n_global : ds->n);
  const int root_candidate = (n_job >= h->cfg.min_examples && 1 < h->cfg.max_depth) ? 1 : 0;
  if (h->num_levels > 0 && h->hist_plan[0].mode == kHistRootSum) YGG_RETURN_IF_ERROR(ensure_root_counts(h));
  const bool hess = hist_hess(h);
  auto slots_of = [&](int l) { return level_slot_bound(h, l); };
  {
    ProfScope ps(h, "grad");
    const LevelBuf lb0 = level_buf(h, h->num_levels > 0 ? slots_of(0) : 0, 1);
    YGG_CUDA(cudaMemsetAsync(lb0.stats, 0, 3 * sizeof(unsigned long long), h->stream));
    QuantParams q{};
    q.n = ds->n; q.n_pad = ds->n_pad; q.g = h->cur_g; q.h = has_h(h) ? h->cur_h : nullptr;
    q.q24 = h->d_q24; q.hq24 = hist_hess(h) ? h->d_hq24 : nullptr;
    q.act = h->d_act; q.act_h = h->d_act_h; q.act_count = h->d_act_count;
    q.node_of_row = h->d_node_of_row; q.st = h->d_st; q.stats = lb0.stats; q.root_candidate = root_candidate;
    q.h_pow2 = h_pow2_of(h);
    q.fixed_g_pow2 = (is_logit(h) && !weighted(h)) ? 1.f : 0.f;
    q.selected = sampling(h) ? h->d_selected : nullptr;
    q.hist_h = weighted(h) ? h->d_weight : nullptr; q.hist_h_pow2 = h->w_pow2;
    k_quantize<<<elementwise_grid(h), 256, 0, h->stream>>>(q);
    h->launches_total++;
// ... 2222 lines not shown
  YGG_CUDA(cudaSetDevice(h->ds->device));
  if (iter >= 0) YGG_RETURN_IF_ERROR(resolve_ties(h, h->trees_done));
  const NodeRec* d_tree = iter >= 0 ? h->d_nodes_all + static_cast<size_t>(iter) * h->max_nodes : h->d_nodes_scratch;
  std::vector<NodeRec> nodes(h->max_nodes);
  YGG_CUDA(cudaMemcpyAsync(nodes.data(), d_tree, sizeof(NodeRec) * h->max_nodes, cudaMemcpyDeviceToHost, h->stream));
  YGG_CUDA(cudaStreamSynchronize(h->stream));
  std::vector<int> stack(1, 0);
  int id = -1;
  for (int k = 0; !stack.empty(); k++) {
    const int i = stack.back();
    stack.pop_back();
    if (k == node) { id = i; break; }
    if (nodes[i].feature >= 0) { stack.push_back(nodes[i].pos_child); stack.push_back(nodes[i].neg_child); }
  }
  if (id < 0) return set_error(YGG_ERR_INVALID_ARGUMENT, "tree %d has no node %d", iter, node);
  const NodeRec& nd = nodes[id];
  if (nd.feature < 0 || nd.cond_type != YGG_FEATURE_CATEGORICAL)
    return set_error(YGG_ERR_INVALID_ARGUMENT, "node %d of tree %d is not a categorical split", node, iter);
  const int wi = h->ds->wide_of.empty() ? -1 : h->ds->wide_of[nd.feature];
  *n_words = wi >= 0 ? (h->ds->wide_bins[wi] + 31) / 32 : 8;
  if (!words || capacity < *n_words) return set_error(YGG_ERR_INVALID_ARGUMENT, "capacity %d < %d words", capacity, *n_words);
  if (wi < 0) {
    std::memcpy(words, nd.mask, sizeof(nd.mask));
    return YGG_OK;
  }
  YGG_CUDA(cudaMemcpyAsync(words, sets_of(h, d_tree) + static_cast<size_t>(id) * h->set_words, sizeof(uint32_t) * *n_words,
                           cudaMemcpyDeviceToHost, h->stream));
  YGG_CUDA(cudaStreamSynchronize(h->stream));
  return YGG_OK;
}

int ygg_gbt_train_loss(ygg_gbt* h, int32_t iter, float* loss, float* secondary) {
  if (!h || !loss || !secondary) return set_error(YGG_ERR_INVALID_ARGUMENT, "null argument");
  if (iter < 0 || iter >= ygg_gbt_num_iterations(h)) return set_error(YGG_ERR_INVALID_ARGUMENT, "iteration %d not logged", iter);
  YGG_CUDA(cudaSetDevice(h->ds->device));
  YGG_RETURN_IF_ERROR(apply_pending(h));
  YGG_RETURN_IF_ERROR(reduce_losses(h));
  LossRec rec;
  YGG_CUDA(cudaMemcpyAsync(&rec, h->d_loss + iter, sizeof(rec), cudaMemcpyDeviceToHost, h->stream));
  YGG_CUDA(cudaStreamSynchronize(h->stream));
  const double n = static_cast<double>(h->shard_mode == kShardRows ? h->n_global : h->ds->n);
  if (user_weighted(h)) *loss = loss_value(h, rec, h->sum_weights, secondary, correct_scale_of(h->w_pow2));
  else *loss = loss_value(h, rec, n, secondary);
  return YGG_OK;
}

int ygg_gbt_get_predictions(ygg_gbt* h, float* out, int64_t n) {
  if (!h || !out) return set_error(YGG_ERR_INVALID_ARGUMENT, "null argument");
  if (n != h->ds->n * h->K) return set_error(YGG_ERR_INVALID_ARGUMENT, "n mismatch (rows x classes expected)");
  YGG_CUDA(cudaSetDevice(h->ds->device));
  YGG_RETURN_IF_ERROR(apply_pending(h));
  YGG_CUDA(cudaMemcpyAsync(out, h->d_pred, n * sizeof(float), cudaMemcpyDeviceToHost, h->stream));
  YGG_CUDA(cudaStreamSynchronize(h->stream));
  return YGG_OK;
}

int ygg_gbt_predict(ygg_gbt* h, const ygg_dataset* ds, float* out, int64_t n) {
  if (!h || !ds || !out) return set_error(YGG_ERR_INVALID_ARGUMENT, "null argument");
  if (ds->device != h->ds->device) return set_error(YGG_ERR_INVALID_ARGUMENT, "the dataset lives on another device");
  if (!same_features(ds, h->ds))
    return set_error(YGG_ERR_INVALID_ARGUMENT, "the dataset does not have the features / binning of the training dataset");
  if (n != ds->n * h->K) return set_error(YGG_ERR_INVALID_ARGUMENT, "n mismatch (rows x classes expected)");
  YGG_CUDA(cudaSetDevice(h->ds->device));
  (void)cudaGetLastError();
  YGG_RETURN_IF_ERROR(resolve_ties(h, h->trees_done));
  float* d_out = nullptr;
  YGG_RETURN_IF_ERROR(dev_alloc(&d_out, static_cast<size_t>(n)));
  const int n_trees = ygg_gbt_num_trees(h);
  float* d_scale = nullptr;
  if (h->dart) {
    const std::vector<float> scale = dart_model_scales(h);
    int st = dev_alloc(&d_scale, scale.size());
    if (st == YGG_OK && !scale.empty() &&
        cudaMemcpyAsync(d_scale, scale.data(), sizeof(float) * scale.size(), cudaMemcpyHostToDevice, h->stream) != cudaSuccess)
      st = set_error(YGG_ERR_CUDA, "upload of the DART weights failed: %s", cudaGetErrorString(cudaGetLastError()));
    if (st != YGG_OK) { dev_free(d_out); dev_free(d_scale); return st; }
  }
  const int grid = static_cast<int>(std::min<int64_t>((ds->n + 255) / 256, static_cast<int64_t>(h->ds->num_sms) * 16));
  auto kernel = h->dart ? k_predict<true> : k_predict<false>;
  kernel<<<grid, 256, 0, h->stream>>>(ds->d_bins, ds->d_wide, ds->d_wide_of, ds->d_num, ds->d_num_of, ds->n, ds->n_pad, h->d_nodes_all, h->d_sets,
                                      h->set_words, pool_nodes(h), h->max_nodes, n_trees, h->K, h->initial_prediction, d_out, d_scale);
  h->launches_total++;
  int st = check_launch("k_predict");
  if (st == YGG_OK && (cudaMemcpyAsync(out, d_out, sizeof(float) * n, cudaMemcpyDeviceToHost, h->stream) != cudaSuccess ||
                       cudaStreamSynchronize(h->stream) != cudaSuccess))
    st = set_error(YGG_ERR_CUDA, "prediction read-back failed: %s", cudaGetErrorString(cudaGetLastError()));
  dev_free(d_out);
  dev_free(d_scale);
  return st;
}

int ygg_gbt_set_predictions(ygg_gbt* h, const float* pred, int64_t n) {
  if (!h || !pred) return set_error(YGG_ERR_INVALID_ARGUMENT, "null argument");
  if (h->dart) return set_error(YGG_ERR_UNIMPLEMENTED, "DART keeps its own accumulator of the predictions: not combined with ygg_gbt_set_predictions");
  if (n != h->ds->n) return set_error(YGG_ERR_INVALID_ARGUMENT, "n mismatch");
  YGG_CUDA(cudaSetDevice(h->ds->device));
  YGG_RETURN_IF_ERROR(apply_pending(h));
  YGG_CUDA(cudaMemcpyAsync(h->d_pred, pred, n * sizeof(float), cudaMemcpyHostToDevice, h->stream));
  YGG_CUDA(cudaStreamSynchronize(h->stream));
  return YGG_OK;
}

int ygg_tree_train_on_gradients(ygg_gbt* h, const float* gradients, const float* hessians, ygg_node* out,
                                int32_t capacity, int32_t* n_nodes) {
  if (!h || !gradients || !out || !n_nodes) return set_error(YGG_ERR_INVALID_ARGUMENT, "null argument");
  if (weighted(h)) return set_error(YGG_ERR_UNIMPLEMENTED, "ygg_tree_train_on_gradients takes unit gradients; not combined with example weights");
  if (has_h(h) && !hessians) return set_error(YGG_ERR_INVALID_ARGUMENT, "hessians required for this loss");
  YGG_CUDA(cudaSetDevice(h->ds->device));
  (void)cudaGetLastError();
  YGG_RETURN_IF_ERROR(apply_pending(h));
  const int64_t n = h->ds->n;
  YGG_CUDA(cudaMemcpyAsync(h->d_g, gradients, n * sizeof(float), cudaMemcpyHostToDevice, h->stream));
  if (has_h(h)) YGG_CUDA(cudaMemcpyAsync(h->d_h, hessians, n * sizeof(float), cudaMemcpyHostToDevice, h->stream));
  const int root_candidate = (n >= h->cfg.min_examples && 1 < h->cfg.max_depth) ? 1 : 0;
  k_begin_iteration<<<1, 1, 0, h->stream>>>(h->d_st, h->d_levels, h->d_fam[0], h->d_slot_node[0], root_candidate);
  h->launches_total++;
  k_absmax<<<elementwise_grid(h), 256, 0, h->stream>>>(h->d_g, n, h->d_st);
  h->launches_total++;
  YGG_RETURN_IF_ERROR(check_launch("k_absmax"));
  h->scratch_tree = false;
  YGG_RETURN_IF_ERROR(grow_tree(h, h->d_nodes_scratch));
  if (h->cfg.growing_strategy == 1) YGG_RETURN_IF_ERROR(best_first_prune(h, h->d_nodes_scratch));
  YGG_RETURN_IF_ERROR(check_device_error(h));
  h->scratch_tree = true;
  std::vector<ygg_node> flat;
  YGG_RETURN_IF_ERROR(fetch_tree(h, h->d_nodes_scratch, &flat, true));
  *n_nodes = static_cast<int32_t>(flat.size());
  if (static_cast<int32_t>(flat.size()) > capacity) return set_error(YGG_ERR_INVALID_ARGUMENT, "capacity %d < %zu nodes", capacity, flat.size());
  std::memcpy(out, flat.data(), flat.size() * sizeof(ygg_node));
  return YGG_OK;
}

int ygg_debug_hist_plan(const ygg_gbt* h, int32_t level, ygg_hist_plan* out) {
  if (!h || !out) return set_error(YGG_ERR_INVALID_ARGUMENT, "null argument");
  if (level < 0 || level >= h->num_levels) return set_error(YGG_ERR_INVALID_ARGUMENT, "level %d outside [0, %d)", level, h->num_levels);
  const HistLaunch& pl = h->hist_plan[level];
  ygg_hist_plan p{};
  if (pl.FL > 0) {
    p.mode = YGG_HIST_HIST2; p.group = pl.FL; p.hist2_tiles = pl.T;
  } else if (pl.SL > 0) {
    p.mode = YGG_HIST_SEGMENTED; p.group = pl.SL;
  } else {
    p.mode = pl.mode == kHistRootSum ? YGG_HIST_ROOT_SUM : pl.mode == kHistPacked ? YGG_HIST_PACKED : YGG_HIST_SHARED;
    p.group = pl.G;
    p.root_lanes = pl.RL;
  }
  p.chunk_blocks = pl.chunk;
  p.slot_window = pl.window;
  p.grid = pl.grid;
  *out = p;
  return YGG_OK;
}

int ygg_debug_level_histogram(ygg_gbt* h, int32_t level, const ygg_hist_plan* plan, const float* gradients,
                              const float* second, const int32_t* slot_of_row, int32_t n_slots, uint64_t* out_sum,
                              uint32_t* out_cnt, uint64_t* out_second, float* out_scales) {
  if (!h || !gradients || !slot_of_row || !out_sum || !out_cnt || !out_scales) return set_error(YGG_ERR_INVALID_ARGUMENT, "null argument");
  if (level < 0 || level >= h->num_levels) return set_error(YGG_ERR_INVALID_ARGUMENT, "level %d outside [0, %d)", level, h->num_levels);
  if (n_slots < 1 || n_slots > 254) return set_error(YGG_ERR_INVALID_ARGUMENT, "n_slots=%d outside [1, 254] (8-bit slots)", n_slots);
  const bool hh = hist_hess(h);
  if (hh != (second != nullptr) || hh != (out_second != nullptr))
    return set_error(YGG_ERR_INVALID_ARGUMENT, hh ? "this handle keeps a second histogram plane: `second` and `out_second` are required"
                                                  : "this handle keeps no second histogram plane: `second` and `out_second` must be NULL");
  const float v_pow2 = hh ? (weighted(h) ? h->w_pow2 : h_pow2_of(h)) : 0.f;
  const int64_t n = h->ds->n;
  bool all_slot0 = true;
  for (int64_t r = 0; r < n; r++) {
    if (!std::isfinite(gradients[r])) return set_error(YGG_ERR_INVALID_ARGUMENT, "gradient of row %lld is not finite", static_cast<long long>(r));
    if (hh && !(second[r] >= 0.f && second[r] <= v_pow2))
      return set_error(YGG_ERR_INVALID_ARGUMENT, "second-plane value of row %lld outside [0, %g]", static_cast<long long>(r), v_pow2);
    if (slot_of_row[r] < -1 || slot_of_row[r] >= n_slots)
      return set_error(YGG_ERR_INVALID_ARGUMENT, "slot %d of row %lld outside [-1, %d)", slot_of_row[r], static_cast<long long>(r), n_slots);
    all_slot0 &= slot_of_row[r] == 0;
  }
  HistLaunch pl{};
  if (plan == nullptr) {
    pl = h->hist_plan[level];
    if (n_slots > level_slot_bound(h, level))
      return set_error(YGG_ERR_INVALID_ARGUMENT, "the plan of level %d holds %d slots, %d requested", level, level_slot_bound(h, level), n_slots);
  } else {
    const ygg_hist_plan& p = *plan;
    if (p.mode < YGG_HIST_ROOT_SUM || p.mode > YGG_HIST_SEGMENTED) return set_error(YGG_ERR_INVALID_ARGUMENT, "unknown mode %d", p.mode);
    const bool root_rows = p.mode == YGG_HIST_ROOT_SUM && p.root_lanes != 0;
    if (root_rows && p.root_lanes != kRootLanes)
      return set_error(YGG_ERR_INVALID_ARGUMENT, "root_lanes=%d: 0 (k_hist) or %d (k_hist_root_rows)", p.root_lanes, kRootLanes);
    const int max_chunk = root_rows ? kRootRowsMaxChunkBlocks : kHistMaxChunkBlocks;
    if (p.chunk_blocks < 1 || p.chunk_blocks > max_chunk)
      return set_error(YGG_ERR_INVALID_ARGUMENT, "chunk_blocks=%d outside [1, %d]", p.chunk_blocks, max_chunk);
    if (p.grid < 1 || p.grid > 65535) return set_error(YGG_ERR_INVALID_ARGUMENT, "grid=%d outside [1, 65535]", p.grid);
    if (p.slot_window < 0) return set_error(YGG_ERR_INVALID_ARGUMENT, "slot_window=%d", p.slot_window);
    pl.chunk = p.chunk_blocks; pl.grid = p.grid;
    if (p.mode == YGG_HIST_HIST2) {
      if (p.group != 8 && p.group != 16 && p.group != 32) return set_error(YGG_ERR_INVALID_ARGUMENT, "k_hist2: %d feature lanes (8, 16 or 32)", p.group);
      if (p.hist2_tiles != 1 && p.hist2_tiles != 2) return set_error(YGG_ERR_INVALID_ARGUMENT, "k_hist2: %d sub-tiles (1 or 2)", p.hist2_tiles);
      if (p.slot_window != 0) return set_error(YGG_ERR_INVALID_ARGUMENT, "k_hist2 has no multi-pass form");
      if (n_slots > 2) return set_error(YGG_ERR_INVALID_ARGUMENT, "k_hist2 with %d slots (at most 2)", n_slots);
      if (hist2_smem_bytes(p.group, n_slots, p.hist2_tiles, level == 0) > kHist2SmemBudget)
        return set_error(YGG_ERR_INVALID_ARGUMENT, "k_hist2 needs %zu bytes of shared memory (budget 216 KB)", hist2_smem_bytes(p.group, n_slots, p.hist2_tiles, level == 0));
      pl.FL = p.group; pl.T = p.hist2_tiles; pl.S = n_slots; pl.G = 1; pl.passes = 1;
      pl.mode = level == 0 ? kHistRootSum : kHistPacked;
    } else if (p.mode == YGG_HIST_SEGMENTED) {
      if (level == 0) return set_error(YGG_ERR_INVALID_ARGUMENT, "k_hist_seg runs below the root only");
      if (hh) return set_error(YGG_ERR_INVALID_ARGUMENT, "a second histogram plane is accumulated by the shared layout only");
      if (p.group != 8 && p.group != 16 && p.group != 32) return set_error(YGG_ERR_INVALID_ARGUMENT, "k_hist_seg: %d feature lanes (8, 16 or 32)", p.group);
      if (p.slot_window != 0) return set_error(YGG_ERR_INVALID_ARGUMENT, "k_hist_seg has no multi-pass form");
      pl.SL = p.group; pl.S = n_slots; pl.G = 1; pl.passes = 1;
      pl.mode = kHistPacked;
    } else if (root_rows) {
      if (p.group != kRootFpl) return set_error(YGG_ERR_INVALID_ARGUMENT, "k_hist_root_rows: group=%d features per lane (%d)", p.group, kRootFpl);
      if (p.slot_window != 0) return set_error(YGG_ERR_INVALID_ARGUMENT, "the root layout has no multi-pass form");
      pl.RL = p.root_lanes; pl.G = p.group; pl.S = n_slots; pl.passes = 1;
      pl.mode = kHistRootSum;
    } else {
      if (p.group < 1 || p.group > 8) return set_error(YGG_ERR_INVALID_ARGUMENT, "k_hist: group=%d outside [1, 8]", p.group);
      pl.mode = p.mode == YGG_HIST_ROOT_SUM ? kHistRootSum : p.mode == YGG_HIST_PACKED ? kHistPacked : kHistShared;
      pl.G = p.group;
      if (p.slot_window > 0) {
        if (pl.mode == kHistRootSum) return set_error(YGG_ERR_INVALID_ARGUMENT, "the root layout has no multi-pass form");
        pl.window = p.slot_window; pl.S = p.slot_window + 1; pl.passes = (n_slots + p.slot_window - 1) / p.slot_window;
      } else {
        pl.S = n_slots; pl.passes = 1;
      }
      size_t budget = 0;
      YGG_RETURN_IF_ERROR(hist_smem_budget(h->ds->device, &budget));
      if (hist_smem_bytes(pl.G, pl.S, hh, pl.mode) > budget)
        return set_error(YGG_ERR_INVALID_ARGUMENT, "k_hist with G=%d and %d slots per pass needs %zu bytes of shared memory (budget %zu)",
                         pl.G, pl.S, hist_smem_bytes(pl.G, pl.S, hh, pl.mode), budget);
    }
  }
  if (hh && (pl.FL > 0 || pl.SL > 0 || pl.RL > 0 || pl.mode != kHistShared))
    return set_error(YGG_ERR_INVALID_ARGUMENT, "a second histogram plane is accumulated by the shared layout only");
  if (pl.mode == kHistRootSum && (level != 0 || sampling(h) || !all_slot0 || n_slots != 1))
    return set_error(YGG_ERR_INVALID_ARGUMENT, "the root layouts need level 0, no row sampling and every row in slot 0");
  if (h->wide_total > 0 && n_slots > h->wide_slots)
    return set_error(YGG_ERR_INVALID_ARGUMENT, "the wide-column planes of this handle hold %d slots, %d requested", h->wide_slots, n_slots);
  YGG_CUDA(cudaSetDevice(h->ds->device));
  (void)cudaGetLastError();
  if (pl.mode == kHistPacked) {
    const int sub = sub_blocks_of(h);
    if (pl.chunk % sub != 0)
      return set_error(YGG_ERR_INVALID_ARGUMENT, "packed layout: chunk_blocks=%d is not a multiple of the %d-block sub-chunk", pl.chunk, sub);
    uint32_t* d_sub = nullptr;
    uint32_t m = 0;
    const int st = chunk_max_count(h, pl.chunk, &d_sub, &m);
    dev_free(d_sub);
    YGG_RETURN_IF_ERROR(st);
    if (m > kPackedMaxUpdates)
      return set_error(YGG_ERR_INVALID_ARGUMENT, "packed layout: a bin receives %u rows in one chunk of %d blocks (at most %u)", m, pl.chunk, kPackedMaxUpdates);
  }
  if (pl.mode == kHistRootSum) YGG_RETURN_IF_ERROR(ensure_root_counts(h));
  YGG_RETURN_IF_ERROR(raise_hist_smem_caps_once(h->ds->device));

  const int64_t n_pad = h->ds->n_pad;
  const int f_hist = h->hist_f_end - h->hist_f_begin;
  std::vector<uint8_t> sel(n), slot8(n);
  for (int64_t r = 0; r < n; r++) {
    sel[r] = slot_of_row[r] >= 0 ? 1 : 0;
    slot8[r] = static_cast<uint8_t>(slot_of_row[r] >= 0 ? slot_of_row[r] : 0);
  }
  std::vector<LevelDesc> lv(32, LevelDesc{0, 0, 0, 0});
  lv[level] = LevelDesc{0, n_slots, n_slots, 0};
  const LevelBuf probe = level_buf(h, n_slots, 1);
  float *d_g = nullptr, *d_v = nullptr;
  uint8_t *d_sel = nullptr, *d_slot = nullptr;
  uint16_t* d_nor = nullptr;
  DeviceState* d_st = nullptr;
  LevelDesc* d_lv = nullptr;
  unsigned long long *d_stats = nullptr, *d_buf = nullptr;
  auto run = [&]() -> int {
    YGG_RETURN_IF_ERROR(dev_alloc(&d_g, n));
    if (hh) YGG_RETURN_IF_ERROR(dev_alloc(&d_v, n));
    YGG_RETURN_IF_ERROR(dev_alloc(&d_sel, n));
    YGG_RETURN_IF_ERROR(dev_alloc(&d_slot, n));
    YGG_RETURN_IF_ERROR(dev_alloc(&d_nor, n_pad));
    YGG_RETURN_IF_ERROR(dev_alloc(&d_st, 1));
    YGG_RETURN_IF_ERROR(dev_alloc(&d_lv, lv.size()));
    YGG_RETURN_IF_ERROR(dev_alloc(&d_stats, 3));
    YGG_RETURN_IF_ERROR(dev_alloc(&d_buf, probe.total_u64));
    YGG_CUDA(cudaMemcpyAsync(d_g, gradients, n * sizeof(float), cudaMemcpyHostToDevice, h->stream));
    if (hh) YGG_CUDA(cudaMemcpyAsync(d_v, second, n * sizeof(float), cudaMemcpyHostToDevice, h->stream));
    YGG_CUDA(cudaMemcpyAsync(d_sel, sel.data(), n, cudaMemcpyHostToDevice, h->stream));
    YGG_CUDA(cudaMemcpyAsync(d_slot, slot8.data(), n, cudaMemcpyHostToDevice, h->stream));
    YGG_CUDA(cudaMemcpyAsync(d_lv, lv.data(), lv.size() * sizeof(LevelDesc), cudaMemcpyHostToDevice, h->stream));
    k_absmax<<<elementwise_grid(h), 256, 0, h->stream>>>(d_g, n, d_st);
    QuantParams q{};
    q.n = n; q.n_pad = n_pad; q.g = d_g; q.h = d_v;
    q.q24 = h->d_q24; q.hq24 = hh ? h->d_hq24 : nullptr;
    q.act = h->d_act; q.act_h = h->d_act_h; q.act_count = h->d_act_count;
    q.node_of_row = d_nor; q.st = d_st; q.stats = d_stats; q.root_candidate = 1;
    q.h_pow2 = hh ? v_pow2 : 1.f;
    k_quantize<<<elementwise_grid(h), 256, 0, h->stream>>>(q);
    YGG_RETURN_IF_ERROR(check_launch("k_quantize"));
    const int cgrid = std::min(h->n_blocks, h->ds->num_sms * 4);
    k_compact_root<<<cgrid, kCompactThreads, 0, h->stream>>>(h->d_act, hh ? h->d_act_h : nullptr, h->d_act_count, h->d_act_sub, d_sel, n,
                                                             h->n_blocks);
    YGG_RETURN_IF_ERROR(check_launch("k_compact_root"));
    k_tag_slots<<<cgrid, 256, 0, h->stream>>>(h->d_act, h->d_act_count, d_slot, h->n_blocks);
    YGG_RETURN_IF_ERROR(check_launch("k_tag_slots"));
    h->launches_total += 4;
    const LevelBuf lb = level_buf(h, n_slots, 1, d_buf);
    YGG_RETURN_IF_ERROR(accumulate_level(h, level, lb, d_lv, pl));
    YGG_RETURN_IF_ERROR(accumulate_wide(h, n_slots));
    std::vector<unsigned long long> buf(lb.total_u64);
    DeviceState st;
    YGG_CUDA(cudaMemcpyAsync(buf.data(), d_buf, lb.total_u64 * sizeof(unsigned long long), cudaMemcpyDeviceToHost, h->stream));
    YGG_CUDA(cudaMemcpyAsync(&st, d_st, sizeof(st), cudaMemcpyDeviceToHost, h->stream));
    YGG_CUDA(cudaStreamSynchronize(h->stream));
    const uint32_t* cnt = reinterpret_cast<const uint32_t*>(buf.data() + (reinterpret_cast<unsigned long long*>(lb.cnt) - d_buf));
    for (int s = 0; s < n_slots; s++)
      for (int f = 0; f < f_hist; f++)
        for (int b = 0; b < kMaxBins; b++) {
          size_t oc;
          const size_t o = slot_hist_offset(s, f, b, lb.f_chunk, static_cast<long long>(lb.chunk_u64), &oc);
          const size_t i = (static_cast<size_t>(s) * f_hist + f) * kMaxBins + b;
          out_sum[i] = buf[o];
          out_cnt[i] = cnt[oc];
          if (hh) out_second[i] = buf[(lb.hsum - d_buf) + o];
        }
    out_scales[0] = st.g_pow2;
    out_scales[1] = v_pow2;
    return YGG_OK;
  };
  const int status = run();
  cudaStreamSynchronize(h->stream);
  dev_free(d_g); dev_free(d_v); dev_free(d_sel); dev_free(d_slot); dev_free(d_nor); dev_free(d_st); dev_free(d_lv);
  dev_free(d_stats); dev_free(d_buf);
  return status;
}

int ygg_debug_wide_histogram(ygg_gbt* h, int32_t n_slots, uint64_t* out_sum, uint32_t* out_cnt, uint64_t* out_second) {
  if (!h || !out_sum || !out_cnt) return set_error(YGG_ERR_INVALID_ARGUMENT, "null argument");
  if (h->wide_total == 0) return set_error(YGG_ERR_INVALID_ARGUMENT, "the handle's dataset has no wide columns");
  if (n_slots < 1 || n_slots > h->wide_slots) return set_error(YGG_ERR_INVALID_ARGUMENT, "n_slots=%d outside [1, %d]", n_slots, h->wide_slots);
  const bool hh = hist_hess(h);
  if (hh != (out_second != nullptr))
    return set_error(YGG_ERR_INVALID_ARGUMENT, hh ? "this handle keeps a second histogram plane: `out_second` is required"
                                                  : "this handle keeps no second histogram plane: `out_second` must be NULL");
  YGG_CUDA(cudaSetDevice(h->ds->device));
  const size_t elems = static_cast<size_t>(n_slots) * h->wide_total;
  YGG_CUDA(cudaMemcpyAsync(out_sum, h->d_wsum, elems * sizeof(uint64_t), cudaMemcpyDeviceToHost, h->stream));
  YGG_CUDA(cudaMemcpyAsync(out_cnt, h->d_wcnt, elems * sizeof(uint32_t), cudaMemcpyDeviceToHost, h->stream));
  if (hh) YGG_CUDA(cudaMemcpyAsync(out_second, h->d_whsum, elems * sizeof(uint64_t), cudaMemcpyDeviceToHost, h->stream));
  YGG_CUDA(cudaStreamSynchronize(h->stream));
  return YGG_OK;
}

int ygg_debug_capture_candidates(ygg_gbt* h, int32_t enabled) {
  if (!h) return set_error(YGG_ERR_INVALID_ARGUMENT, "null handle");
  if (enabled && (h->cfg.candidate_shuffle != 0 || h->cfg.growing_strategy != 0))
    return set_error(YGG_ERR_INVALID_ARGUMENT, "candidate capture covers level-wise trees without the tie-break replay");
  YGG_CUDA(cudaSetDevice(h->ds->device));
  YGG_CUDA(cudaStreamSynchronize(h->stream));
  free_capture(h);
  if (!enabled || h->num_levels == 0) {
    h->cap.on = enabled != 0;
    return YGG_OK;
  }
  ygg_gbt::Capture& c = h->cap;
  const size_t L = static_cast<size_t>(h->num_levels);
  c.f_scan = h->f_end - h->f_begin;
  c.nodes = static_cast<size_t>(1) << std::max(0, h->num_levels - 1);
  const size_t per = c.nodes * c.f_scan;
  int st = dev_alloc(&c.cand, L * per);
  if (st == YGG_OK) st = dev_alloc(&c.mask, L * per * 8);
  if (st == YGG_OK && h->d_wide_thr != nullptr) st = dev_alloc(&c.thr, L * per);
  if (st == YGG_OK && h->d_wide_set != nullptr) {
    c.set_elems = c.nodes * h->ds->n_wide() * h->set_words;
    st = dev_alloc(&c.set, L * c.set_elems);
  }
  if (st == YGG_OK && h->sample_k_valid > 0) st = dev_alloc(&c.tried, L * per);
  if (st == YGG_OK) st = dev_alloc(&c.node_tab, L * h->max_nodes);
  if (st == YGG_OK) st = dev_alloc(&c.fam, L * h->max_level_nodes);
  if (st == YGG_OK) st = dev_alloc(&c.lv, L);
  if (st == YGG_OK) st = dev_alloc(&c.st, 1);
  if (st != YGG_OK) {
    free_capture(h);
    return st;
  }
  c.on = true;
  return YGG_OK;
}

int ygg_debug_level_candidates(ygg_gbt* h, int32_t level, int32_t capacity, ygg_level_node* nodes_out, ygg_candidate* cands,
                               uint32_t* sets, int32_t set_words, int32_t* n_nodes, float* scales) {
  if (!h || !nodes_out || !cands || !n_nodes || !scales) return set_error(YGG_ERR_INVALID_ARGUMENT, "null argument");
  const ygg_gbt::Capture& c = h->cap;
  if (!c.on) return set_error(YGG_ERR_INVALID_ARGUMENT, "candidate capture is not enabled (ygg_debug_capture_candidates)");
  if (c.levels == 0) return set_error(YGG_ERR_INVALID_ARGUMENT, "no tree was grown since candidate capture was enabled");
  if (level < 0 || level >= c.levels) return set_error(YGG_ERR_INVALID_ARGUMENT, "level %d outside [0, %d)", level, c.levels);
  if (sets != nullptr && set_words != h->set_words)
    return set_error(YGG_ERR_INVALID_ARGUMENT, "set_words=%d, the handle's positive sets have %d words", set_words, h->set_words);
  const ygg_dataset* ds = h->ds;
  YGG_CUDA(cudaSetDevice(ds->device));
  const size_t per = c.nodes * c.f_scan;
  LevelDesc lv{};
  DeviceState dst{};
  std::vector<NodeRec> tab(h->max_nodes), tree(h->max_nodes);
  std::vector<Family> fam(h->max_level_nodes);
  std::vector<Candidate> cand(per);
  std::vector<uint32_t> mask(per * 8), set(c.set ? c.set_elems : 0);
  std::vector<float> thr(c.thr ? per : 0), bucket_values(ds->d_bucket_values ? static_cast<size_t>(ds->F) * kMaxBins : 0);
  auto get = [&](void* dst_, const void* src, size_t bytes) {
    return cudaMemcpyAsync(dst_, src, bytes, cudaMemcpyDeviceToHost, h->stream);
  };
  YGG_CUDA(get(&lv, c.lv + level, sizeof(LevelDesc)));
  YGG_CUDA(get(&dst, c.st, sizeof(DeviceState)));
  YGG_CUDA(get(tab.data(), c.node_tab + static_cast<size_t>(level) * h->max_nodes, tab.size() * sizeof(NodeRec)));
  YGG_CUDA(get(tree.data(), c.tree, tree.size() * sizeof(NodeRec)));
  YGG_CUDA(get(fam.data(), c.fam + static_cast<size_t>(level) * h->max_level_nodes, fam.size() * sizeof(Family)));
  YGG_CUDA(get(cand.data(), c.cand + level * per, per * sizeof(Candidate)));
  YGG_CUDA(get(mask.data(), c.mask + level * per * 8, per * 8 * sizeof(uint32_t)));
  if (c.thr) YGG_CUDA(get(thr.data(), c.thr + level * per, per * sizeof(float)));
  if (c.set) YGG_CUDA(get(set.data(), c.set + level * c.set_elems, c.set_elems * sizeof(uint32_t)));
  if (!bucket_values.empty()) YGG_CUDA(get(bucket_values.data(), ds->d_bucket_values, bucket_values.size() * sizeof(float)));
  YGG_CUDA(cudaStreamSynchronize(h->stream));
  *n_nodes = lv.num_nodes;
  if (lv.num_nodes > capacity) return set_error(YGG_ERR_INVALID_ARGUMENT, "capacity %d < %d level nodes", capacity, lv.num_nodes);
  std::vector<int> ids, pre(h->max_nodes, -1);
  preorder_ids(tree, 0, &ids);
  for (size_t i = 0; i < ids.size(); i++) pre[ids[i]] = static_cast<int>(i);
  std::vector<int> derived(lv.num_nodes, 0);
  for (int f = 0; f < lv.num_families; f++)
    if (fam[f].derived >= 0) derived[fam[f].derived - lv.first_node] = 1;
  for (int j = 0; j < lv.num_nodes; j++) {
    const NodeRec& nd = tab[lv.first_node + j];
    nodes_out[j] = ygg_level_node{pre[lv.first_node + j], nd.candidate, derived[j], 0, nd.n};
    for (int fl = 0; fl < c.f_scan; fl++) {
      const size_t ci = static_cast<size_t>(j) * c.f_scan + fl;
      const int fg = h->f_begin + fl;
      const Candidate& k = cand[ci];
      ygg_candidate o{};
      o.lo = o.hi = -1;
      o.threshold_value = std::numeric_limits<float>::quiet_NaN();
      if (nd.candidate && k.found) {
        o.found = 1;
        o.score = k.score;
        o.threshold_bin = thr_bin_of(k.thr);
        o.num_pos_examples = k.n_pos;
        if (k.thr & kThrExactFlag) {
          o.lo = (k.thr >> 9) & 0xFF;
          o.hi = (k.thr >> 17) & 0x1FF;
          o.threshold_value = thr_value_of(k.thr, bucket_values.data() + static_cast<size_t>(fg) * kMaxBins);
        }
        if (!thr.empty() && ((ds->n_wide() > 0 && ds->wide_of[fg] >= 0) || ds->feature_type[fg] == YGG_FEATURE_NUMERICAL))
          o.threshold_value = thr[ci];
        for (int i = 0; i < 8; i++) o.cat_mask[i] = mask[ci * 8 + i];
      }
      cands[ci] = o;
    }
    if (sets != nullptr && c.set != nullptr) {
      const size_t row = static_cast<size_t>(ds->n_wide()) * h->set_words;
      for (size_t i = 0; i < row; i++) sets[j * row + i] = nd.candidate ? set[j * row + i] : 0u;
    }
  }
  scales[0] = dst.g_pow2;
  scales[1] = dst.h_pow2;
  scales[2] = h->w_pow2;
  return YGG_OK;
}

int ygg_partition_rows(ygg_dataset* ds, const uint32_t* rows_in, int64_t n, int32_t feature,
                       int32_t threshold_bin, uint32_t* rows_out, int64_t* n_pos) {
  if (!ds || !rows_in || !rows_out || !n_pos) return set_error(YGG_ERR_INVALID_ARGUMENT, "null argument");
  if (feature < 0 || feature >= ds->F) return set_error(YGG_ERR_INVALID_ARGUMENT, "feature %d out of range", feature);
  if (ds->feature_type[feature] == YGG_FEATURE_NUMERICAL)
    return set_error(YGG_ERR_UNIMPLEMENTED, "feature %d is a presorted numerical column: it has no bins to partition by", feature);
  if (n < 0 || n >= (1ll << 32)) return set_error(YGG_ERR_INVALID_ARGUMENT, "bad row count");
  if (n == 0) { *n_pos = 0; return YGG_OK; }
  for (int64_t i = 0; i < n; i++)
    if (rows_in[i] >= ds->n) return set_error(YGG_ERR_INVALID_ARGUMENT, "row id %u out of range", rows_in[i]);
  YGG_RETURN_IF_ERROR(require_device());
  YGG_CUDA(cudaSetDevice(ds->device));
  (void)cudaGetLastError();
  uint32_t *d_in = nullptr, *d_out = nullptr, *d_cnt = nullptr;
  const int blocks = static_cast<int>((n + 255) / 256);
  YGG_RETURN_IF_ERROR(dev_alloc(&d_in, n));
  YGG_RETURN_IF_ERROR(dev_alloc(&d_out, n));
  YGG_RETURN_IF_ERROR(dev_alloc(&d_cnt, blocks));
  YGG_CUDA(cudaMemcpy(d_in, rows_in, n * sizeof(uint32_t), cudaMemcpyHostToDevice));
// ... 290 lines not shown
```

yggdrasil-decision-forests_b200/csrc/ygg_hist_seg.cuh:

```cuda
#pragma once
#include <cstdint>
#include <type_traits>
#include <cub/block/block_scan.cuh>
#include <cuda_runtime.h>

#include "ygg_device.cuh"
#include "ygg_hist.cuh"

namespace ygg {

constexpr int kSegThreads = 1024;
constexpr int kSegMinBlocks = 1;
constexpr int kSegMinSlots = 4;
constexpr int kSegShallowMinFeatures = 128;
constexpr long long kSegShallowMinElements = 1000000000LL;
constexpr int kSegItemsPerCta = 4;
constexpr int kSegMinPiece = 4096;
constexpr int kSegMaxSlots = 256;
constexpr int kSegScanThreads = 512;

inline int seg_lane_features(int FL, int f_count) { return FL == 32 && f_count > 32 ? 2 : 1; }
inline int seg_min_slots(int f_count, long long rows) {
  return f_count >= kSegShallowMinFeatures && rows * f_count >= kSegShallowMinElements ? 1 : kSegMinSlots;
}
__host__ __device__ inline size_t seg_smem_bytes(int FI) { return static_cast<size_t>(kMaxBins) * 2 * FI * 4; }
__host__ __device__ inline int seg_feature_groups(int FL, int FPL, int f_begin, int f_count) {
  const int off = f_begin & (FPL - 1);
  return (f_count + off + FL * FPL - 1) / (FL * FPL);
}
inline int seg_row_bytes(int F) {
  int b = 32;
  while (b < F && b < 256) b *= 2;
  return b >= F ? b : (F + 255) / 256 * 256;
}

__global__ void __launch_bounds__(256) k_bins_to_rows(const uint8_t* bins, int64_t n_pad, int F, int row_bytes, uint8_t* rows) {
  const int64_t r = static_cast<int64_t>(blockIdx.x) * 256 + threadIdx.x;
  const int f0 = blockIdx.y * 32;
  if (r >= n_pad) return;
  uint32_t w[8] = {0u, 0u, 0u, 0u, 0u, 0u, 0u, 0u};
#pragma unroll
  for (int k = 0; k < 32; k++) {
    const int f = f0 + k;
    const uint32_t v = f < F ? bins[static_cast<int64_t>(f) * n_pad + r] : 0u;
    w[k >> 2] |= v << (8 * (k & 3));
  }
  uint4* dst = reinterpret_cast<uint4*>(rows + r * row_bytes + f0);
  dst[0] = make_uint4(w[0], w[1], w[2], w[3]);
  dst[1] = make_uint4(w[4], w[5], w[6], w[7]);
}

__device__ __forceinline__ uint32_t seg_slot_of(uint2 e, bool valid, uint32_t ns) {
  const uint32_t slot = e.x >> 24;
  return (valid && slot < ns) ? slot : 0xFFFFFFFFu;
}

__global__ void __launch_bounds__(256) k_seg_count(const uint2* act, const int32_t* act_count, int n_blocks, int S,
                                                   const LevelDesc* levels, int level, long long* blk) {
  __shared__ int c[kSegMaxSlots];
  const uint32_t ns = static_cast<uint32_t>(min(S, levels[level].num_slots));
  const int lane = threadIdx.x & 31;
  for (int b = blockIdx.x; b < n_blocks; b += gridDim.x) {
    for (int i = threadIdx.x; i < S; i += blockDim.x) c[i] = 0;
    __syncthreads();
    const int n = act_count[b];
    const uint2* a = act + static_cast<int64_t>(b) * kBlockRows;
    for (int i0 = threadIdx.x & ~31; i0 < n; i0 += blockDim.x) {
      const int i = i0 + lane;
      const uint32_t slot = seg_slot_of(i < n ? __ldg(a + i) : make_uint2(0u, 0u), i < n, ns);
      const uint32_t mask = __match_any_sync(0xFFFFFFFFu, slot);
      if (slot != 0xFFFFFFFFu && (mask & ((1u << lane) - 1u)) == 0u) atomicAdd(&c[slot], __popc(mask));
    }
    __syncthreads();
    for (int i = threadIdx.x; i < S; i += blockDim.x) blk[static_cast<size_t>(i) * n_blocks + b] = c[i];
    __syncthreads();
  }
}

__global__ void __launch_bounds__(kSegScanThreads) k_seg_ranges(const long long* incl, int S, int n_blocks, int chunk_blocks,
                                                                int n_chunks, int target_pieces, long long* seg_off,
                                                                int32_t* piece_start, int32_t* meta) {
  using Scan = cub::BlockScan<long long, kSegScanThreads>;
  __shared__ typename Scan::TempStorage tmp;
  const int tid = threadIdx.x;
  const int R = S * n_chunks;
  const long long total = incl[static_cast<size_t>(S) * n_blocks - 1];
  for (int r = tid; r < R; r += kSegScanThreads) {
    const int s = r / n_chunks, c = r - s * n_chunks;
    const size_t i = static_cast<size_t>(s) * n_blocks + static_cast<size_t>(c) * chunk_blocks;
    seg_off[r] = i == 0 ? 0 : incl[i - 1];
  }
  if (tid == 0) seg_off[R] = total;
  const long long P = max(static_cast<long long>(kSegMinPiece), (total + target_pieces - 1) / target_pieces);
  __syncthreads();
  const int per = (R + kSegScanThreads - 1) / kSegScanThreads;
  const int r0 = min(R, tid * per), r1 = min(R, r0 + per);
  long long pieces = 0;
  for (int r = r0; r < r1; r++) pieces += (seg_off[r + 1] - seg_off[r] + P - 1) / P;
  long long first = 0, n_pieces = 0;
  Scan(tmp).ExclusiveSum(pieces, first, n_pieces);
  for (int r = r0; r < r1; r++) {
    piece_start[r] = static_cast<int32_t>(first);
    first += (seg_off[r + 1] - seg_off[r] + P - 1) / P;
  }
  if (tid == 0) {
    piece_start[R] = static_cast<int32_t>(n_pieces);
    meta[0] = static_cast<int32_t>(P);
    meta[1] = static_cast<int32_t>(n_pieces);
    meta[2] = 0;
  }
}

__global__ void __launch_bounds__(256) k_seg_scatter(const uint2* act, const int32_t* act_count, int n_blocks, int S,
                                                     const LevelDesc* levels, int level, const long long* incl, uint2* seg) {
  __shared__ int cnt[8][kSegMaxSlots];
  __shared__ long long cur[8][kSegMaxSlots];
  const int warp = threadIdx.x >> 5, lane = threadIdx.x & 31;
  const uint32_t ns = static_cast<uint32_t>(min(S, levels[level].num_slots));
  const uint32_t lt = (1u << lane) - 1u;
  for (int b = blockIdx.x; b < n_blocks; b += gridDim.x) {
    for (int s = lane; s < static_cast<int>(ns); s += 32) cnt[warp][s] = 0;
    __syncwarp();
    const int n = act_count[b];
    const int part = (n + 8 * 32 - 1) / (8 * 32) * 32;
    const int e0 = min(n, warp * part), e1 = min(n, e0 + part);
    const uint2* a = act + static_cast<int64_t>(b) * kBlockRows;
    for (int i0 = e0; i0 < e1; i0 += 32) {
      const int i = i0 + lane;
      const uint32_t slot = seg_slot_of(i < e1 ? __ldg(a + i) : make_uint2(0u, 0u), i < e1, ns);
      const uint32_t mask = __match_any_sync(0xFFFFFFFFu, slot);
      if (slot != 0xFFFFFFFFu && (mask & lt) == 0u) cnt[warp][slot] += __popc(mask);
      __syncwarp();
    }
    __syncthreads();
    for (int s = threadIdx.x; s < static_cast<int>(ns); s += blockDim.x) {
      const size_t gi = static_cast<size_t>(s) * n_blocks + b;
      long long o = gi == 0 ? 0 : incl[gi - 1];
#pragma unroll
      for (int w = 0; w < 8; w++) {
        cur[w][s] = o;
        o += cnt[w][s];
      }
    }
    __syncthreads();
    const uint32_t row0 = static_cast<uint32_t>(b) * kBlockRows;
    for (int i0 = e0; i0 < e1; i0 += 32) {
      const int i = i0 + lane;
      const uint2 e = i < e1 ? __ldg(a + i) : make_uint2(0u, 0u);
      const uint32_t slot = seg_slot_of(e, i < e1, ns);
      const uint32_t mask = __match_any_sync(0xFFFFFFFFu, slot);
      const int rank = __popc(mask & lt);
      long long o = 0;
      if (slot != 0xFFFFFFFFu) o = cur[warp][slot];
      __syncwarp();
      if (slot != 0xFFFFFFFFu && rank == 0) cur[warp][slot] = o + __popc(mask);
      __syncwarp();
      if (slot != 0xFFFFFFFFu) seg[o + rank] = make_uint2(e.x, row0 + e.y);
    }
    __syncthreads();
  }
}

template <int FPL>
__device__ __forceinline__ uint32_t ldg_row(const uint8_t* p) {
  uint32_t v;
  if constexpr (FPL == 2) asm("ld.global.nc.L2::256B.u16 %0, [%1];" : "=r"(v) : "l"(p));
  else asm("ld.global.nc.L2::256B.u8 %0, [%1];" : "=r"(v) : "l"(p));
  return v;
}

struct SegParams {
  const uint8_t* rows;
  uint32_t row_bytes;
  const uint2* seg;
  const long long* seg_off;
  const int32_t* piece_start;
  int32_t* meta;
  int n_ranges, n_chunks;
  int f_begin, f_count;
  unsigned long long* hist_sum;
  uint32_t* hist_cnt;
  int f_chunk;
  long long chunk_stride;
};

template <int FL, int FPL>
__global__ void __launch_bounds__(kSegThreads, kSegMinBlocks) k_hist_seg(SegParams p) {
  static_assert(FL == 8 || FL == 16 || FL == 32, "feature lanes");
  static_assert(FPL == 1 || (FPL == 2 && FL == 32), "two features per lane at 32 lanes only");
  constexpr int FI = FL * FPL;
  constexpr int R = 32 / FL;
  constexpr int kSteps = 32 / R;
  constexpr int kInFlight = FL == 32 ? 32 : 8;
  constexpr int kWarps = kSegThreads / 32;
  constexpr int kWords = kMaxBins * 2 * FI;
  constexpr uint32_t kBinBytes = 2u * FI * 4u, kPlaneBytes = FI * 4u, kHalfBytes = FL * 4u;
  extern __shared__ __align__(16) uint32_t s_bins[];
  __shared__ int s_item;
  const int tid = threadIdx.x, lane = tid & 31, warp = tid >> 5;
  const int fl = lane % FL, sub = lane / FL;
  uint32_t s_base = static_cast<uint32_t>(__cvta_generic_to_shared(s_bins));
  asm volatile("mov.u32 %0, %0;" : "+r"(s_base));
  const int off = FPL == 2 ? (p.f_begin & 1) : 0;
  const int n_fg = seg_feature_groups(FL, FPL, p.f_begin, p.f_count);
  const int P = p.meta[0];
  const int n_items = p.meta[1] * n_fg;
  for (int i = tid; i < kWords; i += kSegThreads) s_bins[i] = 0u;
  const uint32_t a_lane = s_base + static_cast<uint32_t>(fl) * 4u;
  for (;;) {
    if (tid == 0) s_item = atomicAdd(&p.meta[2], 1);
    __syncthreads();
    const int item = s_item;
    if (item >= n_items) break;
    const int piece = item / n_fg, fg = item - piece * n_fg;
    int lo = 0, hi = p.n_ranges;
    while (hi - lo > 1) {
      const int mid = (lo + hi) >> 1;
      if (__ldg(p.piece_start + mid) <= piece) lo = mid;
      else hi = mid;
    }
    const long long beg = __ldg(p.seg_off + lo) + static_cast<long long>(piece - __ldg(p.piece_start + lo)) * P;
    const int len = static_cast<int>(min(static_cast<long long>(P), __ldg(p.seg_off + lo + 1) - beg));
    const int slot = lo / p.n_chunks;
    const int f0 = fg * FI - off;
    const int last = min(FI, p.f_count - f0) - 1;
    const uint8_t* col = p.rows + p.f_begin + f0 + min(fl * FPL, last & ~(FPL - 1));
    const uint2* sp = p.seg + beg;

    int e = warp * 32;
    uint2 cur = e + lane < len ? __ldg(sp + e + lane) : make_uint2(0u, 0u);
    for (; e < len; e += kWarps * 32) {
      const int en = e + kWarps * 32 + lane;
      const uint2 nxt = en < len ? __ldg(sp + en) : make_uint2(0u, 0u);
      const uint32_t xq = e + lane < len ? ((cur.x & kQMax) | 0x80000000u) : 0u;
#pragma unroll
      for (int j0 = 0; j0 < kSteps; j0 += kInFlight) {
        uint32_t b[kInFlight];
#pragma unroll
        for (int j = 0; j < kInFlight; j++) {
          const uint32_t row = __shfl_sync(0xFFFFFFFFu, cur.y, (j0 + j) * R + sub);
          b[j] = ldg_row<FPL>(col + static_cast<size_t>(row) * p.row_bytes);
        }
#pragma unroll
        for (int j = 0; j < kInFlight; j++) {
          const uint32_t x = __shfl_sync(0xFFFFFFFFu, xq, (j0 + j) * R + sub);
          const uint32_t inc = (((x >> kPackedCoarseShift) & 0x3Fu) << kPackedCntBits) | (x >> 31), q = x & kQMax;
          const uint32_t a = a_lane + (FPL == 2 ? b[j] & 0xFFu : b[j]) * kBinBytes;
          smem_red(a, inc);
          smem_red(a + kPlaneBytes, q);
          if constexpr (FPL == 2) {
            const uint32_t a1 = a_lane + kHalfBytes + (b[j] >> 8) * kBinBytes;
            smem_red(a1, inc);
            smem_red(a1 + kPlaneBytes, q);
          }
        }
      }
      cur = nxt;
    }
    __syncthreads();

    constexpr int QL = FI >= 16 ? 4 : 2;
    constexpr int TB = 32 / QL;
    constexpr int kQuadGroups = FI / (4 * QL);
    constexpr int kTiles = kMaxBins / TB * kQuadGroups;
    const int tr = lane / QL, tq = lane % QL;
    for (int t = warp; t < kTiles; t += kWarps) {
      const int bin = t / kQuadGroups * TB + tr;
      const int k0 = (t % kQuadGroups * QL + tq) * 4;
      uint4* w = reinterpret_cast<uint4*>(s_bins + bin * 2 * FI + k0);
      const uint4 c4 = w[0], l4 = w[FI / 4];
      w[0] = make_uint4(0u, 0u, 0u, 0u);
      w[FI / 4] = make_uint4(0u, 0u, 0u, 0u);
      const uint32_t cs[4] = {c4.x, c4.y, c4.z, c4.w}, ls[4] = {l4.x, l4.y, l4.z, l4.w};
#pragma unroll
      for (int j = 0; j < 4; j++) {
        const int k = k0 + j;
        const int f = f0 + (k % FL) * FPL + k / FL;
        const uint32_t c = cs[j];
        if (c == 0u || f < 0 || f >= p.f_count) continue;
        size_t oc;
        const size_t o = slot_hist_offset(slot, f, bin, p.f_chunk, p.chunk_stride, &oc);
        const unsigned long long base = static_cast<unsigned long long>(c >> kPackedCntBits) << kPackedCoarseShift;
        atomicAdd(&p.hist_sum[o], base + static_cast<uint32_t>(ls[j] - static_cast<uint32_t>(base)));
        atomicAdd(&p.hist_cnt[oc], c & kPackedMaxUpdates);
      }
    }
  }
}

}
```

Before: 168.7.

## Fuse segmented-histogram count, scan, ranges and scatter into one cooperative kernel

Replaces the four-step segment layout pipeline (count kernel, CUB device scan, single-CTA range kernel, scatter kernel) with a single cooperative kernel that uses grid.sync. Each CTA owns a contiguous range of blocks and stores packed 16-bit per-warp prefixes. The per-slot CTA totals are scanned across the grid, then seg_off and the piece layout are computed and the rows are scattered. The aim is to remove launch overhead and the single-CTA scan bottleneck, and loads are batched four at a time. The cost is the grid-wide barriers, a grid size tied to occupancy, and a debug entry point for the new layout.

```diff
diff --git a/include/ygg_b200.h b/include/ygg_b200.h
--- a/include/ygg_b200.h
+++ b/include/ygg_b200.h
@@ -216,6 +216,11 @@
                               const float* second, const int32_t* slot_of_row, int32_t n_slots, uint64_t* out_sum,
                               uint32_t* out_cnt, uint64_t* out_second, float* out_scales);
 
+int ygg_debug_seg_layout(ygg_gbt* h, int32_t level, const ygg_hist_plan* plan, const float* gradients,
+                         const int32_t* slot_of_row, int32_t n_slots, int32_t level_slots, uint32_t* out_act,
+                         int32_t* out_act_count, uint32_t* out_seg, int64_t* out_seg_off, int32_t* out_piece_start,
+                         int32_t* out_meta);
+
 int ygg_debug_wide_histogram(ygg_gbt* h, int32_t n_slots, uint64_t* out_sum, uint32_t* out_cnt, uint64_t* out_second);
 
 int ygg_debug_capture_candidates(ygg_gbt* h, int32_t enabled);
diff --git a/yggdrasil-decision-forests_b200/_capi.py b/yggdrasil-decision-forests_b200/_capi.py
--- a/yggdrasil-decision-forests_b200/_capi.py
+++ b/yggdrasil-decision-forests_b200/_capi.py
@@ -92,6 +92,7 @@
     "ygg_num_candidate_attributes", "ygg_candidate_key", "ygg_gbt_set_candidate_sampling", "ygg_debug_level_tried",
     "ygg_gbt_set_dart", "ygg_gbt_get_dart_weights", "ygg_gbt_get_dart_dropped",
     "ygg_dataset_set_wide_discretized_column", "ygg_dataset_builder_add_numerical16_async", "ygg_discretize_boundaries16",
+    "ygg_debug_seg_layout",
 ]
 
 
@@ -676,6 +677,29 @@
                                               ptr(s2, C.c_uint64), ptr(scales, C.c_float)))
         return s, c, s2, (float(scales[0]), float(scales[1]))
 
+    def seg_layout(self, level, g, slot_of_row, n_slots, level_slots=None, plan=None):
+        g = np.ascontiguousarray(g, dtype=np.float32)
+        slots = np.ascontiguousarray(slot_of_row, dtype=np.int32)
+        n_blocks = -(-len(g) // 8192)
+        if plan is None:
+            chunk = self.hist_plan(level).chunk_blocks
+        else:
+            chunk = plan.chunk_blocks
+        R = int(n_slots) * -(-n_blocks // max(1, chunk))
+        act = np.zeros((n_blocks, 8192, 2), np.uint32)
+        act_count = np.zeros(n_blocks, np.int32)
+        seg = np.zeros((len(g), 2), np.uint32)
+        seg_off = np.zeros(R + 1, np.int64)
+        piece_start = np.zeros(R + 1, np.int32)
+        meta = np.zeros(3, np.int32)
+        check(lib().ygg_debug_seg_layout(self.handle, C.c_int32(level), None if plan is None else C.byref(plan),
+                                         ptr(g, C.c_float), ptr(slots, C.c_int32), C.c_int32(n_slots),
+                                         C.c_int32(n_slots if level_slots is None else level_slots), ptr(act, C.c_uint32),
+                                         ptr(act_count, C.c_int32), ptr(seg, C.c_uint32), ptr(seg_off, C.c_int64),
+                                         ptr(piece_start, C.c_int32), ptr(meta, C.c_int32)))
+        return {"act": act, "act_count": act_count, "seg": seg[:int(seg_off[-1])].copy(), "seg_off": seg_off,
+                "piece_start": piece_start, "meta": meta}
+
     def wide_histogram(self, n_slots):
         total = sum(nb for nb, _ in getattr(self.dataset, "wide", {}).values())
         s = np.zeros((int(n_slots), total), np.uint64)
diff --git a/yggdrasil-decision-forests_b200/csrc/ygg_engine.cu b/yggdrasil-decision-forests_b200/csrc/ygg_engine.cu
--- a/yggdrasil-decision-forests_b200/csrc/ygg_engine.cu
+++ b/yggdrasil-decision-forests_b200/csrc/ygg_engine.cu
@@ -284,12 +284,12 @@
   HistLaunch hist_plan[32]{};
   int part_smem_children = 0;
   uint2* d_hseg = nullptr;
-  long long* d_hseg_blk = nullptr;
   long long* d_hseg_off = nullptr;
   int32_t* d_hseg_piece = nullptr;
   int32_t* d_hseg_meta = nullptr;
-  void* d_hseg_temp = nullptr;
-  size_t hseg_temp_bytes = 0;
+  uint4* d_hseg_blk = nullptr;
+  long long* d_hseg_cta = nullptr;
+  int seg_group_grid = 0;
   bool profiling = false;
   std::map<std::string, ProfileSlot> profile;
   std::vector<std::pair<std::string, std::pair<cudaEvent_t, cudaEvent_t>>> pending_events;
@@ -351,8 +351,9 @@
   h->pending_events.clear();
 }
 
-int check_launch(const char* what) {
-  cudaError_t e = cudaGetLastError();
+int check_launch(const char* what, cudaError_t launched = cudaSuccess) {
+  const cudaError_t last = cudaGetLastError();
+  const cudaError_t e = launched != cudaSuccess ? launched : last;
   if (e != cudaSuccess) return set_error(YGG_ERR_CUDA, "launch of %s failed: %s", what, cudaGetErrorString(e));
   return YGG_OK;
 }
@@ -926,27 +927,29 @@
 }
 
 void free_seg_buffers(ygg_gbt* h) {
-  dev_free(h->d_hseg); dev_free(h->d_hseg_blk); dev_free(h->d_hseg_off); dev_free(h->d_hseg_piece); dev_free(h->d_hseg_meta);
-  dev_free(h->d_hseg_temp);
-  h->d_hseg = nullptr; h->d_hseg_blk = nullptr; h->d_hseg_off = nullptr; h->d_hseg_piece = nullptr; h->d_hseg_meta = nullptr;
-  h->d_hseg_temp = nullptr;
-  h->hseg_temp_bytes = 0;
+  dev_free(h->d_hseg); dev_free(h->d_hseg_off); dev_free(h->d_hseg_piece); dev_free(h->d_hseg_meta);
+  dev_free(h->d_hseg_blk); dev_free(h->d_hseg_cta);
+  h->d_hseg = nullptr; h->d_hseg_off = nullptr; h->d_hseg_piece = nullptr; h->d_hseg_meta = nullptr;
+  h->d_hseg_blk = nullptr; h->d_hseg_cta = nullptr;
+  h->seg_group_grid = 0;
 }
 int ensure_seg_buffers(ygg_gbt* h) {
-  if (h->d_hseg_temp != nullptr) return YGG_OK;
+  if (h->d_hseg_cta != nullptr) return YGG_OK;
   const size_t ranges = static_cast<size_t>(kSegMaxSlots) * h->n_blocks;
   auto alloc_all = [&]() -> int {
+    int per_sm = 0;
+    YGG_CUDA(cudaOccupancyMaxActiveBlocksPerMultiprocessor(&per_sm, k_seg_group, kSegGroupThreads, 0));
+    if (per_sm < 1) return set_error(YGG_ERR_CUDA, "k_seg_group: no CTA fits on an SM");
+    const int max_grid = std::min(h->n_blocks, per_sm * h->ds->num_sms);
+    const int per = (h->n_blocks + max_grid - 1) / max_grid;
+    const int grid = (h->n_blocks + per - 1) / per;
     YGG_RETURN_IF_ERROR(dev_alloc(&h->d_hseg, static_cast<size_t>(h->ds->n_pad)));
-    YGG_RETURN_IF_ERROR(dev_alloc(&h->d_hseg_blk, ranges));
     YGG_RETURN_IF_ERROR(dev_alloc(&h->d_hseg_off, ranges + 1));
     YGG_RETURN_IF_ERROR(dev_alloc(&h->d_hseg_piece, ranges + 1));
     YGG_RETURN_IF_ERROR(dev_alloc(&h->d_hseg_meta, 4));
-    size_t temp_bytes = 0;
-    YGG_CUDA(cub::DeviceScan::InclusiveSum(nullptr, temp_bytes, h->d_hseg_blk, h->d_hseg_blk, static_cast<int>(ranges)));
-    char* temp = nullptr;
-    YGG_RETURN_IF_ERROR(dev_alloc(&temp, temp_bytes));
-    h->hseg_temp_bytes = temp_bytes;
-    h->d_hseg_temp = temp;
+    YGG_RETURN_IF_ERROR(dev_alloc(&h->d_hseg_blk, ranges));
+    YGG_RETURN_IF_ERROR(dev_alloc(&h->d_hseg_cta, static_cast<size_t>(kSegMaxSlots) * (grid + 1)));
+    h->seg_group_grid = grid;
     return YGG_OK;
   };
   const int st = alloc_all();
@@ -954,26 +957,32 @@
   return st;
 }
 
+int group_level_seg(ygg_gbt* h, int l, const LevelDesc* levels, const HistLaunch& pl) {
+  YGG_RETURN_IF_ERROR(ensure_seg_buffers(h));
+  const int f_count = h->hist_f_end - h->hist_f_begin;
+  const int fpl = seg_lane_features(pl.SL, f_count);
+  const int n_fg = seg_feature_groups(pl.SL, fpl, h->hist_f_begin, f_count);
+  SegGroupParams gp{};
+  gp.act = h->d_act; gp.act_count = h->d_act_count; gp.n_blocks = h->n_blocks; gp.S = pl.S;
+  gp.levels = levels; gp.level = l;
+  gp.chunk_blocks = pl.chunk; gp.n_chunks = (h->n_blocks + pl.chunk - 1) / pl.chunk;
+  gp.target_pieces = std::max(1, (kSegItemsPerCta * pl.grid + n_fg - 1) / n_fg);
+  gp.blk = h->d_hseg_blk; gp.cta = h->d_hseg_cta;
+  gp.seg = h->d_hseg; gp.seg_off = h->d_hseg_off; gp.piece_start = h->d_hseg_piece; gp.meta = h->d_hseg_meta;
+  void* args[] = {&gp};
+  const cudaError_t e = cudaLaunchCooperativeKernel(reinterpret_cast<const void*>(k_seg_group), dim3(h->seg_group_grid),
+                                                    dim3(kSegGroupThreads), args, 0, h->stream);
+  h->launches_total++;
+  return check_launch("k_seg_group", e);
+}
+
 int launch_hist_seg(ygg_gbt* h, int l, const LevelBuf& lb, const LevelDesc* levels, const HistLaunch& pl) {
   ygg_dataset* ds = h->ds;
   YGG_RETURN_IF_ERROR(ensure_bins_rows(ds));
-  YGG_RETURN_IF_ERROR(ensure_seg_buffers(h));
+  YGG_RETURN_IF_ERROR(group_level_seg(h, l, levels, pl));
   const int f_count = h->hist_f_end - h->hist_f_begin;
   const int n_chunks = (h->n_blocks + pl.chunk - 1) / pl.chunk;
   const int fpl = seg_lane_features(pl.SL, f_count);
-  const int n_fg = seg_feature_groups(pl.SL, fpl, h->hist_f_begin, f_count);
-  const int target_pieces = std::max(1, (kSegItemsPerCta * pl.grid + n_fg - 1) / n_fg);
-  k_seg_count<<<std::min(h->n_blocks, ds->num_sms * 8), 256, 0, h->stream>>>(h->d_act, h->d_act_count, h->n_blocks, pl.S,
-                                                                               levels, l, h->d_hseg_blk);
-  YGG_RETURN_IF_ERROR(check_launch("k_seg_count"));
-  YGG_CUDA(cub::DeviceScan::InclusiveSum(h->d_hseg_temp, h->hseg_temp_bytes, h->d_hseg_blk, h->d_hseg_blk, pl.S * h->n_blocks,
-                                         h->stream));
-  k_seg_ranges<<<1, kSegScanThreads, 0, h->stream>>>(h->d_hseg_blk, pl.S, h->n_blocks, pl.chunk, n_chunks, target_pieces,
-                                                     h->d_hseg_off, h->d_hseg_piece, h->d_hseg_meta);
-  YGG_RETURN_IF_ERROR(check_launch("k_seg_ranges"));
-  k_seg_scatter<<<std::min(h->n_blocks, ds->num_sms * 8), 256, 0, h->stream>>>(h->d_act, h->d_act_count, h->n_blocks, pl.S, levels, l,
-                                                               h->d_hseg_blk, h->d_hseg);
-  YGG_RETURN_IF_ERROR(check_launch("k_seg_scatter"));
   SegParams sp{};
   sp.rows = ds->d_bins_rows; sp.row_bytes = static_cast<uint32_t>(seg_row_bytes(ds->F));
   sp.seg = h->d_hseg; sp.seg_off = h->d_hseg_off; sp.piece_start = h->d_hseg_piece; sp.meta = h->d_hseg_meta;
@@ -986,7 +995,7 @@
   else if (pl.SL == 32) k_hist_seg<32, 1><<<pl.grid, kSegThreads, smem, h->stream>>>(sp);
   else if (pl.SL == 16) k_hist_seg<16, 1><<<pl.grid, kSegThreads, smem, h->stream>>>(sp);
   else k_hist_seg<8, 1><<<pl.grid, kSegThreads, smem, h->stream>>>(sp);
-  h->launches_total += 5;
+  h->launches_total++;
   return check_launch("k_hist_seg");
 }
 
@@ -3515,6 +3524,65 @@
   return YGG_OK;
 }
 
+namespace {
+struct DebugLevelInputs {
+  ygg_gbt* h;
+  float *d_g = nullptr, *d_v = nullptr;
+  uint8_t *d_sel = nullptr, *d_slot = nullptr;
+  uint16_t* d_nor = nullptr;
+  DeviceState* d_st = nullptr;
+  LevelDesc* d_lv = nullptr;
+  unsigned long long* d_stats = nullptr;
+  explicit DebugLevelInputs(ygg_gbt* h_) : h(h_) {}
+  ~DebugLevelInputs() {
+    cudaStreamSynchronize(h->stream);
+    dev_free(d_g); dev_free(d_v); dev_free(d_sel); dev_free(d_slot); dev_free(d_nor); dev_free(d_st); dev_free(d_lv);
+    dev_free(d_stats);
+  }
+  int fill(int level, int num_slots, const float* gradients, const float* second, float v_pow2, const int32_t* slot_of_row) {
+    const int64_t n = h->ds->n, n_pad = h->ds->n_pad;
+    const bool hh = second != nullptr;
+    std::vector<uint8_t> sel(n), slot8(n);
+    for (int64_t r = 0; r < n; r++) {
+      sel[r] = slot_of_row[r] >= 0 ? 1 : 0;
+      slot8[r] = static_cast<uint8_t>(slot_of_row[r] >= 0 ? slot_of_row[r] : 0);
+    }
+    std::vector<LevelDesc> lv(32, LevelDesc{0, 0, 0, 0});
+    lv[level] = LevelDesc{0, num_slots, num_slots, 0};
+    YGG_RETURN_IF_ERROR(dev_alloc(&d_g, n));
+    if (hh) YGG_RETURN_IF_ERROR(dev_alloc(&d_v, n));
+    YGG_RETURN_IF_ERROR(dev_alloc(&d_sel, n));
+    YGG_RETURN_IF_ERROR(dev_alloc(&d_slot, n));
+    YGG_RETURN_IF_ERROR(dev_alloc(&d_nor, n_pad));
+    YGG_RETURN_IF_ERROR(dev_alloc(&d_st, 1));
+    YGG_RETURN_IF_ERROR(dev_alloc(&d_lv, lv.size()));
+    YGG_RETURN_IF_ERROR(dev_alloc(&d_stats, 3));
+    YGG_CUDA(cudaMemcpyAsync(d_g, gradients, n * sizeof(float), cudaMemcpyHostToDevice, h->stream));
+    if (hh) YGG_CUDA(cudaMemcpyAsync(d_v, second, n * sizeof(float), cudaMemcpyHostToDevice, h->stream));
+    YGG_CUDA(cudaMemcpyAsync(d_sel, sel.data(), n, cudaMemcpyHostToDevice, h->stream));
+    YGG_CUDA(cudaMemcpyAsync(d_slot, slot8.data(), n, cudaMemcpyHostToDevice, h->stream));
+    YGG_CUDA(cudaMemcpyAsync(d_lv, lv.data(), lv.size() * sizeof(LevelDesc), cudaMemcpyHostToDevice, h->stream));
+    k_absmax<<<elementwise_grid(h), 256, 0, h->stream>>>(d_g, n, d_st);
+    QuantParams q{};
+    q.n = n; q.n_pad = n_pad; q.g = d_g; q.h = d_v;
+    q.q24 = h->d_q24; q.hq24 = hh ? h->d_hq24 : nullptr;
+    q.act = h->d_act; q.act_h = h->d_act_h; q.act_count = h->d_act_count;
+    q.node_of_row = d_nor; q.st = d_st; q.stats = d_stats; q.root_candidate = 1;
+    q.h_pow2 = hh ? v_pow2 : 1.f;
+    k_quantize<<<elementwise_grid(h), 256, 0, h->stream>>>(q);
+    YGG_RETURN_IF_ERROR(check_launch("k_quantize"));
+    const int cgrid = std::min(h->n_blocks, h->ds->num_sms * 4);
+    k_compact_root<<<cgrid, kCompactThreads, 0, h->stream>>>(h->d_act, hh ? h->d_act_h : nullptr, h->d_act_count, h->d_act_sub, d_sel, n,
+                                                             h->n_blocks);
+    YGG_RETURN_IF_ERROR(check_launch("k_compact_root"));
+    k_tag_slots<<<cgrid, 256, 0, h->stream>>>(h->d_act, h->d_act_count, d_slot, h->n_blocks);
+    YGG_RETURN_IF_ERROR(check_launch("k_tag_slots"));
+    h->launches_total += 4;
+    return YGG_OK;
+  }
+};
+}
+
 int ygg_debug_level_histogram(ygg_gbt* h, int32_t level, const ygg_hist_plan* plan, const float* gradients,
                               const float* second, const int32_t* slot_of_row, int32_t n_slots, uint64_t* out_sum,
                               uint32_t* out_cnt, uint64_t* out_second, float* out_scales) {
@@ -3614,60 +3682,20 @@
   if (pl.mode == kHistRootSum) YGG_RETURN_IF_ERROR(ensure_root_counts(h));
   YGG_RETURN_IF_ERROR(raise_hist_smem_caps_once(h->ds->device));
 
-  const int64_t n_pad = h->ds->n_pad;
   const int f_hist = h->hist_f_end - h->hist_f_begin;
-  std::vector<uint8_t> sel(n), slot8(n);
-  for (int64_t r = 0; r < n; r++) {
-    sel[r] = slot_of_row[r] >= 0 ? 1 : 0;
-    slot8[r] = static_cast<uint8_t>(slot_of_row[r] >= 0 ? slot_of_row[r] : 0);
-  }
-  std::vector<LevelDesc> lv(32, LevelDesc{0, 0, 0, 0});
-  lv[level] = LevelDesc{0, n_slots, n_slots, 0};
   const LevelBuf probe = level_buf(h, n_slots, 1);
-  float *d_g = nullptr, *d_v = nullptr;
-  uint8_t *d_sel = nullptr, *d_slot = nullptr;
-  uint16_t* d_nor = nullptr;
-  DeviceState* d_st = nullptr;
-  LevelDesc* d_lv = nullptr;
-  unsigned long long *d_stats = nullptr, *d_buf = nullptr;
+  DebugLevelInputs in(h);
+  unsigned long long* d_buf = nullptr;
   auto run = [&]() -> int {
-    YGG_RETURN_IF_ERROR(dev_alloc(&d_g, n));
-    if (hh) YGG_RETURN_IF_ERROR(dev_alloc(&d_v, n));
-    YGG_RETURN_IF_ERROR(dev_alloc(&d_sel, n));
-    YGG_RETURN_IF_ERROR(dev_alloc(&d_slot, n));
-    YGG_RETURN_IF_ERROR(dev_alloc(&d_nor, n_pad));
-    YGG_RETURN_IF_ERROR(dev_alloc(&d_st, 1));
-    YGG_RETURN_IF_ERROR(dev_alloc(&d_lv, lv.size()));
-    YGG_RETURN_IF_ERROR(dev_alloc(&d_stats, 3));
+    YGG_RETURN_IF_ERROR(in.fill(level, n_slots, gradients, second, v_pow2, slot_of_row));
     YGG_RETURN_IF_ERROR(dev_alloc(&d_buf, probe.total_u64));
-    YGG_CUDA(cudaMemcpyAsync(d_g, gradients, n * sizeof(float), cudaMemcpyHostToDevice, h->stream));
-    if (hh) YGG_CUDA(cudaMemcpyAsync(d_v, second, n * sizeof(float), cudaMemcpyHostToDevice, h->stream));
-    YGG_CUDA(cudaMemcpyAsync(d_sel, sel.data(), n, cudaMemcpyHostToDevice, h->stream));
-    YGG_CUDA(cudaMemcpyAsync(d_slot, slot8.data(), n, cudaMemcpyHostToDevice, h->stream));
-    YGG_CUDA(cudaMemcpyAsync(d_lv, lv.data(), lv.size() * sizeof(LevelDesc), cudaMemcpyHostToDevice, h->stream));
-    k_absmax<<<elementwise_grid(h), 256, 0, h->stream>>>(d_g, n, d_st);
-    QuantParams q{};
-    q.n = n; q.n_pad = n_pad; q.g = d_g; q.h = d_v;
-    q.q24 = h->d_q24; q.hq24 = hh ? h->d_hq24 : nullptr;
-    q.act = h->d_act; q.act_h = h->d_act_h; q.act_count = h->d_act_count;
-    q.node_of_row = d_nor; q.st = d_st; q.stats = d_stats; q.root_candidate = 1;
-    q.h_pow2 = hh ? v_pow2 : 1.f;
-    k_quantize<<<elementwise_grid(h), 256, 0, h->stream>>>(q);
-    YGG_RETURN_IF_ERROR(check_launch("k_quantize"));
-    const int cgrid = std::min(h->n_blocks, h->ds->num_sms * 4);
-    k_compact_root<<<cgrid, kCompactThreads, 0, h->stream>>>(h->d_act, hh ? h->d_act_h : nullptr, h->d_act_count, h->d_act_sub, d_sel, n,
-                                                             h->n_blocks);
-    YGG_RETURN_IF_ERROR(check_launch("k_compact_root"));
-    k_tag_slots<<<cgrid, 256, 0, h->stream>>>(h->d_act, h->d_act_count, d_slot, h->n_blocks);
-    YGG_RETURN_IF_ERROR(check_launch("k_tag_slots"));
-    h->launches_total += 4;
     const LevelBuf lb = level_buf(h, n_slots, 1, d_buf);
-    YGG_RETURN_IF_ERROR(accumulate_level(h, level, lb, d_lv, pl));
+    YGG_RETURN_IF_ERROR(accumulate_level(h, level, lb, in.d_lv, pl));
     YGG_RETURN_IF_ERROR(accumulate_wide(h, n_slots));
     std::vector<unsigned long long> buf(lb.total_u64);
     DeviceState st;
     YGG_CUDA(cudaMemcpyAsync(buf.data(), d_buf, lb.total_u64 * sizeof(unsigned long long), cudaMemcpyDeviceToHost, h->stream));
-    YGG_CUDA(cudaMemcpyAsync(&st, d_st, sizeof(st), cudaMemcpyDeviceToHost, h->stream));
+    YGG_CUDA(cudaMemcpyAsync(&st, in.d_st, sizeof(st), cudaMemcpyDeviceToHost, h->stream));
     YGG_CUDA(cudaStreamSynchronize(h->stream));
     const uint32_t* cnt = reinterpret_cast<const uint32_t*>(buf.data() + (reinterpret_cast<unsigned long long*>(lb.cnt) - d_buf));
     for (int s = 0; s < n_slots; s++)
@@ -3686,8 +3714,64 @@
   };
   const int status = run();
   cudaStreamSynchronize(h->stream);
-  dev_free(d_g); dev_free(d_v); dev_free(d_sel); dev_free(d_slot); dev_free(d_nor); dev_free(d_st); dev_free(d_lv);
-  dev_free(d_stats); dev_free(d_buf);
+  dev_free(d_buf);
+  return status;
+}
+
+int ygg_debug_seg_layout(ygg_gbt* h, int32_t level, const ygg_hist_plan* plan, const float* gradients,
+                         const int32_t* slot_of_row, int32_t n_slots, int32_t level_slots, uint32_t* out_act,
+                         int32_t* out_act_count, uint32_t* out_seg, int64_t* out_seg_off, int32_t* out_piece_start,
+                         int32_t* out_meta) {
+  if (!h || !gradients || !slot_of_row || !out_seg || !out_seg_off || !out_piece_start || !out_meta)
+    return set_error(YGG_ERR_INVALID_ARGUMENT, "null argument");
+  if (level < 1 || level >= h->num_levels) return set_error(YGG_ERR_INVALID_ARGUMENT, "level %d outside [1, %d): k_hist_seg runs below the root only", level, h->num_levels);
+  if (n_slots < 1 || n_slots > kSegMaxSlots) return set_error(YGG_ERR_INVALID_ARGUMENT, "n_slots=%d outside [1, %d] (8-bit slots)", n_slots, kSegMaxSlots);
+  if (level_slots < 0 || level_slots > n_slots) return set_error(YGG_ERR_INVALID_ARGUMENT, "level_slots=%d outside [0, %d]", level_slots, n_slots);
+  if (hist_hess(h)) return set_error(YGG_ERR_INVALID_ARGUMENT, "a second histogram plane is accumulated by the shared layout only");
+  const int64_t n = h->ds->n;
+  for (int64_t r = 0; r < n; r++) {
+    if (!std::isfinite(gradients[r])) return set_error(YGG_ERR_INVALID_ARGUMENT, "gradient of row %lld is not finite", static_cast<long long>(r));
+    if (slot_of_row[r] < -1 || slot_of_row[r] >= kSegMaxSlots)
+      return set_error(YGG_ERR_INVALID_ARGUMENT, "slot %d of row %lld outside [-1, %d)", slot_of_row[r], static_cast<long long>(r), kSegMaxSlots);
+  }
+  HistLaunch pl{};
+  if (plan == nullptr) {
+    pl = h->hist_plan[level];
+    if (pl.SL == 0) return set_error(YGG_ERR_INVALID_ARGUMENT, "the plan of level %d is not k_hist_seg's", level);
+    if (n_slots > level_slot_bound(h, level))
+      return set_error(YGG_ERR_INVALID_ARGUMENT, "the plan of level %d holds %d slots, %d requested", level, level_slot_bound(h, level), n_slots);
+  } else {
+    const ygg_hist_plan& p = *plan;
+    if (p.mode != YGG_HIST_SEGMENTED) return set_error(YGG_ERR_INVALID_ARGUMENT, "mode %d: the layout is k_hist_seg's (YGG_HIST_SEGMENTED)", p.mode);
+    if (p.group != 8 && p.group != 16 && p.group != 32) return set_error(YGG_ERR_INVALID_ARGUMENT, "k_hist_seg: %d feature lanes (8, 16 or 32)", p.group);
+    if (p.chunk_blocks < 1 || p.chunk_blocks > kHistMaxChunkBlocks)
+      return set_error(YGG_ERR_INVALID_ARGUMENT, "chunk_blocks=%d outside [1, %d]", p.chunk_blocks, kHistMaxChunkBlocks);
+    if (p.grid < 1 || p.grid > 65535) return set_error(YGG_ERR_INVALID_ARGUMENT, "grid=%d outside [1, 65535]", p.grid);
+    if (p.slot_window != 0) return set_error(YGG_ERR_INVALID_ARGUMENT, "k_hist_seg has no multi-pass form");
+    pl.SL = p.group; pl.chunk = p.chunk_blocks; pl.grid = p.grid; pl.G = 1; pl.passes = 1; pl.mode = kHistPacked;
+  }
+  pl.S = n_slots;
+  YGG_CUDA(cudaSetDevice(h->ds->device));
+  (void)cudaGetLastError();
+  const int n_chunks = (h->n_blocks + pl.chunk - 1) / pl.chunk;
+  const size_t R = static_cast<size_t>(n_slots) * n_chunks;
+  DebugLevelInputs in(h);
+  auto run = [&]() -> int {
+    YGG_RETURN_IF_ERROR(in.fill(level, level_slots, gradients, nullptr, 0.f, slot_of_row));
+    YGG_RETURN_IF_ERROR(group_level_seg(h, level, in.d_lv, pl));
+    YGG_CUDA(cudaMemcpyAsync(out_seg_off, h->d_hseg_off, (R + 1) * sizeof(int64_t), cudaMemcpyDeviceToHost, h->stream));
+    YGG_CUDA(cudaMemcpyAsync(out_piece_start, h->d_hseg_piece, (R + 1) * sizeof(int32_t), cudaMemcpyDeviceToHost, h->stream));
+    YGG_CUDA(cudaMemcpyAsync(out_meta, h->d_hseg_meta, 3 * sizeof(int32_t), cudaMemcpyDeviceToHost, h->stream));
+    if (out_act) YGG_CUDA(cudaMemcpyAsync(out_act, h->d_act, static_cast<size_t>(h->n_blocks) * kBlockRows * sizeof(uint2), cudaMemcpyDeviceToHost, h->stream));
+    if (out_act_count) YGG_CUDA(cudaMemcpyAsync(out_act_count, h->d_act_count, h->n_blocks * sizeof(int32_t), cudaMemcpyDeviceToHost, h->stream));
+    YGG_CUDA(cudaStreamSynchronize(h->stream));
+    const int64_t total = out_seg_off[R];
+    if (total < 0 || total > n) return set_error(YGG_ERR_CUDA, "k_seg_group: %lld entries for %lld rows", static_cast<long long>(total), static_cast<long long>(n));
+    YGG_CUDA(cudaMemcpy(out_seg, h->d_hseg, static_cast<size_t>(total) * sizeof(uint2), cudaMemcpyDeviceToHost));
+    return YGG_OK;
+  };
+  const int status = run();
+  cudaStreamSynchronize(h->stream);
   return status;
 }
 
diff --git a/yggdrasil-decision-forests_b200/csrc/ygg_hist_seg.cuh b/yggdrasil-decision-forests_b200/csrc/ygg_hist_seg.cuh
--- a/yggdrasil-decision-forests_b200/csrc/ygg_hist_seg.cuh
+++ b/yggdrasil-decision-forests_b200/csrc/ygg_hist_seg.cuh
@@ -1,6 +1,7 @@
 #pragma once
 #include <cstdint>
 #include <type_traits>
+#include <cooperative_groups.h>
 #include <cub/block/block_scan.cuh>
 #include <cuda_runtime.h>
 
@@ -17,7 +18,6 @@
 constexpr int kSegItemsPerCta = 4;
 constexpr int kSegMinPiece = 4096;
 constexpr int kSegMaxSlots = 256;
-constexpr int kSegScanThreads = 512;
 
 inline int seg_lane_features(int FL, int f_count) { return FL == 32 && f_count > 32 ? 2 : 1; }
 inline int seg_min_slots(int f_count, long long rows) {
@@ -55,107 +55,163 @@
   return (valid && slot < ns) ? slot : 0xFFFFFFFFu;
 }
 
-__global__ void __launch_bounds__(256) k_seg_count(const uint2* act, const int32_t* act_count, int n_blocks, int S,
-                                                   const LevelDesc* levels, int level, long long* blk) {
-  __shared__ int c[kSegMaxSlots];
-  const uint32_t ns = static_cast<uint32_t>(min(S, levels[level].num_slots));
-  const int lane = threadIdx.x & 31;
-  for (int b = blockIdx.x; b < n_blocks; b += gridDim.x) {
-    for (int i = threadIdx.x; i < S; i += blockDim.x) c[i] = 0;
-    __syncthreads();
-    const int n = act_count[b];
-    const uint2* a = act + static_cast<int64_t>(b) * kBlockRows;
-    for (int i0 = threadIdx.x & ~31; i0 < n; i0 += blockDim.x) {
-      const int i = i0 + lane;
-      const uint32_t slot = seg_slot_of(i < n ? __ldg(a + i) : make_uint2(0u, 0u), i < n, ns);
-      const uint32_t mask = __match_any_sync(0xFFFFFFFFu, slot);
-      if (slot != 0xFFFFFFFFu && (mask & ((1u << lane) - 1u)) == 0u) atomicAdd(&c[slot], __popc(mask));
-    }
-    __syncthreads();
-    for (int i = threadIdx.x; i < S; i += blockDim.x) blk[static_cast<size_t>(i) * n_blocks + b] = c[i];
-    __syncthreads();
-  }
-}
-
-__global__ void __launch_bounds__(kSegScanThreads) k_seg_ranges(const long long* incl, int S, int n_blocks, int chunk_blocks,
-                                                                int n_chunks, int target_pieces, long long* seg_off,
-                                                                int32_t* piece_start, int32_t* meta) {
-  using Scan = cub::BlockScan<long long, kSegScanThreads>;
-  __shared__ typename Scan::TempStorage tmp;
-  const int tid = threadIdx.x;
-  const int R = S * n_chunks;
-  const long long total = incl[static_cast<size_t>(S) * n_blocks - 1];
-  for (int r = tid; r < R; r += kSegScanThreads) {
-    const int s = r / n_chunks, c = r - s * n_chunks;
-    const size_t i = static_cast<size_t>(s) * n_blocks + static_cast<size_t>(c) * chunk_blocks;
-    seg_off[r] = i == 0 ? 0 : incl[i - 1];
-  }
-  if (tid == 0) seg_off[R] = total;
-  const long long P = max(static_cast<long long>(kSegMinPiece), (total + target_pieces - 1) / target_pieces);
-  __syncthreads();
-  const int per = (R + kSegScanThreads - 1) / kSegScanThreads;
-  const int r0 = min(R, tid * per), r1 = min(R, r0 + per);
-  long long pieces = 0;
-  for (int r = r0; r < r1; r++) pieces += (seg_off[r + 1] - seg_off[r] + P - 1) / P;
-  long long first = 0, n_pieces = 0;
-  Scan(tmp).ExclusiveSum(pieces, first, n_pieces);
-  for (int r = r0; r < r1; r++) {
-    piece_start[r] = static_cast<int32_t>(first);
-    first += (seg_off[r + 1] - seg_off[r] + P - 1) / P;
-  }
-  if (tid == 0) {
-    piece_start[R] = static_cast<int32_t>(n_pieces);
-    meta[0] = static_cast<int32_t>(P);
-    meta[1] = static_cast<int32_t>(n_pieces);
-    meta[2] = 0;
-  }
-}
-
-__global__ void __launch_bounds__(256) k_seg_scatter(const uint2* act, const int32_t* act_count, int n_blocks, int S,
-                                                     const LevelDesc* levels, int level, const long long* incl, uint2* seg) {
-  __shared__ int cnt[8][kSegMaxSlots];
-  __shared__ long long cur[8][kSegMaxSlots];
-  const int warp = threadIdx.x >> 5, lane = threadIdx.x & 31;
-  const uint32_t ns = static_cast<uint32_t>(min(S, levels[level].num_slots));
+constexpr int kSegGroupThreads = 256;
+constexpr int kSegGroupParts = kSegGroupThreads / 32;
+constexpr int kSegGroupMinBlocks = 5;
+constexpr int kSegGroupBatch = 4;
+static_assert(kSegMaxSlots == kSegGroupThreads, "one slot per thread");
+static_assert(kBlockRows < 65536, "a block's per-slot prefixes are 16-bit");
+
+struct SegGroupParams {
+  const uint2* act;
+  const int32_t* act_count;
+  int n_blocks, S;
+  const LevelDesc* levels;
+  int level;
+  int chunk_blocks, n_chunks, target_pieces;
+  uint4* blk;
+  long long* cta;
+  uint2* seg;
+  long long* seg_off;
+  int32_t* piece_start;
+  int32_t* meta;
+};
+
+__global__ void __launch_bounds__(kSegGroupThreads, kSegGroupMinBlocks) k_seg_group(SegGroupParams p) {
+  using Scan = cub::BlockScan<long long, kSegGroupThreads>;
+  __shared__ union {
+    int cnt[kSegGroupParts][kSegMaxSlots];
+    long long cur[kSegGroupParts][kSegMaxSlots];
+    typename Scan::TempStorage scan;
+  } sm;
+  cooperative_groups::grid_group grid = cooperative_groups::this_grid();
+  const int tid = threadIdx.x, warp = tid >> 5, lane = tid & 31, s = tid;
   const uint32_t lt = (1u << lane) - 1u;
-  for (int b = blockIdx.x; b < n_blocks; b += gridDim.x) {
-    for (int s = lane; s < static_cast<int>(ns); s += 32) cnt[warp][s] = 0;
-    __syncwarp();
-    const int n = act_count[b];
-    const int part = (n + 8 * 32 - 1) / (8 * 32) * 32;
+  const int S = p.S, G = gridDim.x, c = blockIdx.x;
+  const uint32_t ns = static_cast<uint32_t>(min(S, p.levels[p.level].num_slots));
+  const int per = (p.n_blocks + G - 1) / G;
+  const int b0 = min(p.n_blocks, c * per), b1 = min(p.n_blocks, b0 + per);
+
+  long long tot = 0;
+  for (int b = b0; b < b1; b++) {
+#pragma unroll
+    for (int w = 0; w < kSegGroupParts; w++) sm.cnt[w][s] = 0;
+    __syncthreads();
+    const int n = __ldg(p.act_count + b);
+    const int part = (n + kSegGroupThreads - 1) / kSegGroupThreads * 32;
     const int e0 = min(n, warp * part), e1 = min(n, e0 + part);
-    const uint2* a = act + static_cast<int64_t>(b) * kBlockRows;
-    for (int i0 = e0; i0 < e1; i0 += 32) {
-      const int i = i0 + lane;
-      const uint32_t slot = seg_slot_of(i < e1 ? __ldg(a + i) : make_uint2(0u, 0u), i < e1, ns);
-      const uint32_t mask = __match_any_sync(0xFFFFFFFFu, slot);
-      if (slot != 0xFFFFFFFFu && (mask & lt) == 0u) cnt[warp][slot] += __popc(mask);
-      __syncwarp();
-    }
-    __syncthreads();
-    for (int s = threadIdx.x; s < static_cast<int>(ns); s += blockDim.x) {
-      const size_t gi = static_cast<size_t>(s) * n_blocks + b;
-      long long o = gi == 0 ? 0 : incl[gi - 1];
-#pragma unroll
-      for (int w = 0; w < 8; w++) {
-        cur[w][s] = o;
-        o += cnt[w][s];
-      }
-    }
-    __syncthreads();
+    const uint2* a = p.act + static_cast<int64_t>(b) * kBlockRows;
+    for (int i0 = e0; i0 < e1; i0 += 32 * kSegGroupBatch) {
+      uint2 ev[kSegGroupBatch];
+#pragma unroll
+      for (int j = 0; j < kSegGroupBatch; j++) ev[j] = i0 + 32 * j + lane < e1 ? __ldg(a + i0 + 32 * j + lane) : make_uint2(0u, 0u);
+#pragma unroll
+      for (int j = 0; j < kSegGroupBatch; j++) {
+        const uint32_t slot = seg_slot_of(ev[j], i0 + 32 * j + lane < e1, ns);
+        const uint32_t mask = __match_any_sync(0xFFFFFFFFu, slot);
+        if (slot != 0xFFFFFFFFu && (mask & lt) == 0u) sm.cnt[warp][slot] += __popc(mask);
+        __syncwarp();
+      }
+    }
+    __syncthreads();
+    if (s < S) {
+      uint32_t pre[kSegGroupParts], o = 0;
+#pragma unroll
+      for (int w = 0; w < kSegGroupParts; w++) {
+        pre[w] = o;
+        o += static_cast<uint32_t>(sm.cnt[w][s]);
+      }
+      p.blk[static_cast<size_t>(b) * S + s] =
+          make_uint4(pre[1] | pre[2] << 16, pre[3] | pre[4] << 16, pre[5] | pre[6] << 16, pre[7] | o << 16);
+      tot += o;
+    }
+  }
+  if (s < S) p.cta[static_cast<size_t>(s) * G + c] = tot;
+  grid.sync();
+
+  for (int t = c; t < S; t += G) {
+    long long* row = p.cta + static_cast<size_t>(t) * G;
+    long long carry = 0;
+    for (int k0 = 0; k0 < G; k0 += kSegGroupThreads) {
+      const int k = k0 + tid;
+      const long long v = k < G ? __ldcg(row + k) : 0;
+      long long x, agg;
+      Scan(sm.scan).ExclusiveSum(v, x, agg);
+      if (k < G) row[k] = carry + x;
+      carry += agg;
+      __syncthreads();
+    }
+    if (tid == 0) p.cta[static_cast<size_t>(S) * G + t] = carry;
+  }
+  grid.sync();
+
+  long long base = 0, total = 0;
+  Scan(sm.scan).ExclusiveSum(s < S ? __ldcg(p.cta + static_cast<size_t>(S) * G + s) : 0LL, base, total);
+  const long long start = s < S ? base + __ldcg(p.cta + static_cast<size_t>(s) * G + c) : 0;
+  if (s < S) {
+    long long o = start;
+    for (int b = b0; b < b1; b++) {
+      if (b % p.chunk_blocks == 0) p.seg_off[static_cast<size_t>(s) * p.n_chunks + b / p.chunk_blocks] = o;
+      o += __ldcg(p.blk + static_cast<size_t>(b) * S + s).w >> 16;
+    }
+  }
+  const int R = S * p.n_chunks;
+  if (c == 0 && tid == 0) p.seg_off[R] = total;
+  grid.sync();
+
+  if (c == G - 1) {
+    const long long P = max(static_cast<long long>(kSegMinPiece), (total + p.target_pieces - 1) / p.target_pieces);
+    const int rpt = (R + kSegGroupThreads - 1) / kSegGroupThreads;
+    const int r0 = min(R, tid * rpt), r1 = min(R, r0 + rpt);
+    long long pieces = 0;
+    for (int r = r0; r < r1; r++) pieces += (__ldcg(p.seg_off + r + 1) - __ldcg(p.seg_off + r) + P - 1) / P;
+    long long first = 0, n_pieces = 0;
+    Scan(sm.scan).ExclusiveSum(pieces, first, n_pieces);
+    for (int r = r0; r < r1; r++) {
+      p.piece_start[r] = static_cast<int32_t>(first);
+      first += (__ldcg(p.seg_off + r + 1) - __ldcg(p.seg_off + r) + P - 1) / P;
+    }
+    if (tid == 0) {
+      p.piece_start[R] = static_cast<int32_t>(n_pieces);
+      p.meta[0] = static_cast<int32_t>(P);
+      p.meta[1] = static_cast<int32_t>(n_pieces);
+      p.meta[2] = 0;
+    }
+    __syncthreads();
+  }
+
+  long long o = start;
+  for (int b = b0; b < b1; b++) {
+    if (s < S) {
+      const uint4 q = __ldcg(p.blk + static_cast<size_t>(b) * S + s);
+      const uint32_t pre[kSegGroupParts] = {0u, q.x & 0xFFFFu, q.x >> 16, q.y & 0xFFFFu, q.y >> 16, q.z & 0xFFFFu, q.z >> 16,
+                                            q.w & 0xFFFFu};
+#pragma unroll
+      for (int w = 0; w < kSegGroupParts; w++) sm.cur[w][s] = o + pre[w];
+      o += q.w >> 16;
+    }
+    __syncthreads();
+    const int n = __ldg(p.act_count + b);
+    const int part = (n + kSegGroupThreads - 1) / kSegGroupThreads * 32;
+    const int e0 = min(n, warp * part), e1 = min(n, e0 + part);
+    const uint2* a = p.act + static_cast<int64_t>(b) * kBlockRows;
     const uint32_t row0 = static_cast<uint32_t>(b) * kBlockRows;
-    for (int i0 = e0; i0 < e1; i0 += 32) {
-      const int i = i0 + lane;
-      const uint2 e = i < e1 ? __ldg(a + i) : make_uint2(0u, 0u);
-      const uint32_t slot = seg_slot_of(e, i < e1, ns);
-      const uint32_t mask = __match_any_sync(0xFFFFFFFFu, slot);
-      const int rank = __popc(mask & lt);
-      long long o = 0;
-      if (slot != 0xFFFFFFFFu) o = cur[warp][slot];
-      __syncwarp();
-      if (slot != 0xFFFFFFFFu && rank == 0) cur[warp][slot] = o + __popc(mask);
-      __syncwarp();
-      if (slot != 0xFFFFFFFFu) seg[o + rank] = make_uint2(e.x, row0 + e.y);
+    for (int i0 = e0; i0 < e1; i0 += 32 * kSegGroupBatch) {
+      uint2 ev[kSegGroupBatch];
+#pragma unroll
+      for (int j = 0; j < kSegGroupBatch; j++) ev[j] = i0 + 32 * j + lane < e1 ? __ldg(a + i0 + 32 * j + lane) : make_uint2(0u, 0u);
+#pragma unroll
+      for (int j = 0; j < kSegGroupBatch; j++) {
+        const uint32_t slot = seg_slot_of(ev[j], i0 + 32 * j + lane < e1, ns);
+        const uint32_t mask = __match_any_sync(0xFFFFFFFFu, slot);
+        const int rank = __popc(mask & lt);
+        long long d = 0;
+        if (slot != 0xFFFFFFFFu) d = sm.cur[warp][slot];
+        __syncwarp();
+        if (slot != 0xFFFFFFFFu && rank == 0) sm.cur[warp][slot] = d + __popc(mask);
+        __syncwarp();
+        if (slot != 0xFFFFFFFFu) p.seg[d + rank] = make_uint2(ev[j].x, row0 + ev[j].y);
+      }
     }
     __syncthreads();
   }
```

Result: faster. 173.0 (median of 6 runs) (+2.6%).
